# BAMresearch/PGDrome

Measured on AMD Instinct MI355X. Metric: PGD fixed-point iters/sec + SpMV HBM GB/s, 256^3 P1 space x 1D param, higher is better.
Workload: dtype f64

## Files before the change

### include/pgd_amd.h

```cpp
#ifndef PGD_AMD_H
#define PGD_AMD_H

#include <stdint.h>

#ifdef __cplusplus
extern "C" {
#endif

typedef int64_t pgd_handle;

enum {
    PGD_OK = 0,
    PGD_ERR_INVALID = -1,
    PGD_ERR_HIP = -2,
    PGD_ERR_NOMEM = -3,
    PGD_ERR_LIMIT = -4,
    PGD_ERR_SINGULAR = -5,
    PGD_ERR_NODEVICE = -6,
    PGD_ERR_TIMEOUT = -7,
    PGD_ERR_PEER = -8
};

enum {
    PGD_ATOM_MASS = 0,
// ... 89 lines not shown
int pgd_slots_upload(pgd_handle ctx, const double *in, int first, int count);
int pgd_flags_reset(pgd_handle ctx);
int pgd_flags_download(pgd_handle ctx, int32_t *done, int32_t *iters, int32_t *status);
int pgd_op_diag_inv(pgd_handle ctx, pgd_handle op, pgd_handle dinv);
int pgd_op_symmetrize(pgd_handle ctx, pgd_handle op, int *used);
int pgd_atom_product_form(pgd_handle ctx, pgd_handle A, int *form);

int pgd_op_classify(pgd_handle ctx, pgd_handle op, int *classes);
int pgd_spmv_dot_slot(pgd_handle ctx, pgd_handle A, pgd_handle x, pgd_handle y, pgd_handle w,
                      int64_t r0, int64_t r1, int slot);
int pgd_pcg_init_slot(pgd_handle ctx, pgd_handle b, pgd_handle q, pgd_handle dinv, pgd_handle r,
                      pgd_handle z, pgd_handle p, int64_t r0, int64_t r1, int slot);
int pgd_pcg_tol_slot(pgd_handle ctx, double rtol, double atol, int slot_rr, int slot_bb,
                     int slot_tol2);
int pgd_pcg_xr_slot(pgd_handle ctx, pgd_handle x, pgd_handle r, pgd_handle p, pgd_handle q,
                    pgd_handle dinv, pgd_handle z, int64_t r0, int64_t r1, int slot_rz,
                    int slot_pq, int slot_out);
int pgd_pcg_check_slot(pgd_handle ctx, int slot_rr, int slot_tol2);
int pgd_pcg_p_slot(pgd_handle ctx, pgd_handle p, pgd_handle z, int64_t r0, int64_t r1,
                   int slot_num, int slot_den);

int pgd_cg_init_slot(pgd_handle ctx, pgd_handle b, pgd_handle q, pgd_handle dinv, pgd_handle r,
                     pgd_handle u, pgd_handle p, pgd_handle s, int64_t r0, int64_t r1, int base);
int pgd_cg_update_slot(pgd_handle ctx, pgd_handle x, pgd_handle r, pgd_handle u, pgd_handle w,
                       pgd_handle p, pgd_handle s, pgd_handle dinv, int64_t r0, int64_t r1, int base);
int pgd_cg_scalars_slot(pgd_handle ctx, int base, int init, double rtol, double atol);

typedef int (*pgd_halo_fn)(void *user, pgd_handle vec, int64_t own0, int64_t own1, int64_t lo_ghost,
                           int64_t hi_ghost);
typedef int (*pgd_allreduce_fn)(void *user, int first_slot, int count);
int pgd_comm_bind_callbacks(pgd_handle ctx, pgd_halo_fn halo, pgd_allreduce_fn allreduce, void *user,
                            int rank, int world);
int pgd_comm_unique_id(pgd_handle ctx, uint8_t *out128);
int pgd_comm_bind_rccl(pgd_handle ctx, const uint8_t *id128, int rank, int world);
int pgd_comm_overlap(pgd_handle ctx, int mode, int *state);
int pgd_comm_unbind(pgd_handle ctx);
int pgd_comm_timeout(pgd_handle ctx, double seconds);
int pgd_comm_prof(pgd_handle ctx, int mode, double *out8);
int pgd_comm_info(pgd_handle ctx, int *kind , int *rank, int *world);
int pgd_comm_halo(pgd_handle ctx, pgd_handle vec, int64_t own0, int64_t own1, int64_t lo_ghost,
                  int64_t hi_ghost);
int pgd_comm_allreduce_slots(pgd_handle ctx, int first_slot, int count);

#define PGD_PUSH_BLOB_BYTES 256
int pgd_comm_push_export(pgd_handle ctx, int64_t n, int64_t own0, int64_t own1, int64_t lo_ghost, int64_t hi_ghost,
                         uint8_t *blob );
int pgd_comm_push_attach(pgd_handle ctx, const uint8_t *lower_blob, const uint8_t *upper_blob, int *state);
int pgd_comm_push(pgd_handle ctx, int mode, int *state);
int pgd_comm_allreduce_attach(pgd_handle ctx, const uint8_t *all_blobs, int *state);
int pgd_comm_allreduce_direct(pgd_handle ctx, int mode, int *state);
int pgd_pcg_solve_sharded(pgd_handle ctx, pgd_handle A, pgd_handle b, pgd_handle x, int64_t own0,
                          int64_t own1, int64_t lo_ghost, int64_t hi_ghost, double rtol, double atol,
                          int maxit, int *iters, double *rel_res);

int pgd_bicgstab_solve(pgd_handle ctx, pgd_handle A, pgd_handle b, pgd_handle x, double rtol, double atol,
                       int maxit, int *iters, double *rel_res);

int pgd_start_gram(pgd_handle ctx, pgd_handle A, const pgd_handle *vecs, int k, pgd_handle b, int64_t r0,
                   int64_t r1, double *out);
int pgd_start_residual(pgd_handle ctx, pgd_handle A, int k, const double *coefs, pgd_handle b, pgd_handle r);

int pgd_vec_multidot(pgd_handle ctx, pgd_handle x, const pgd_handle *ys, int k, int64_t lo, int64_t hi,
                     double *out);

int pgd_vec_multidot_pair(pgd_handle ctx, pgd_handle x0, pgd_handle x1, const pgd_handle *ys, int k, int64_t lo,
                          int64_t hi, double *out);

enum { PGD_BLOCK_F32 = 0, PGD_BLOCK_F64 = 1 };
int pgd_block_create(pgd_handle ctx, int64_t n, int k, int dtype, pgd_handle *block);
int pgd_block_free(pgd_handle ctx, pgd_handle block);
int pgd_block_info(pgd_handle ctx, pgd_handle block, int64_t *n, int *k, int *dtype, int64_t *bytes);
int pgd_block_storage(pgd_handle ctx, int *dtype);
int pgd_block_set_column(pgd_handle ctx, pgd_handle block, int j, pgd_handle vec);
int pgd_block_get_column(pgd_handle ctx, pgd_handle block, int j, pgd_handle vec);
int pgd_block_dots(pgd_handle ctx, pgd_handle block, pgd_handle vec_r, int64_t lo, int64_t hi, double *out);
int pgd_block_combine(pgd_handle ctx, pgd_handle block, const double *coefs, pgd_handle vec_base_or_0, pgd_handle vec_x);

enum { PGD_EVAL_STATS = 1, PGD_EVAL_ENVELOPE = 2, PGD_EVAL_EXCEED = 4, PGD_EVAL_FIELDS = 8 };
int pgd_eval_batch(pgd_handle ctx, const pgd_handle *modes, int k, const double *coefs, int64_t s, int want,
                   double threshold, double *sample_stats, pgd_handle env_min, pgd_handle env_max, pgd_handle exceed,
                   pgd_handle fields);

enum {
    PGD_TUNE_BLOCK_STORAGE = 54,
    PGD_TUNE_PCG_RECOMPUTE_Q = 53,
    PGD_TUNE_EVAL_SAMPLE_CHUNK = 52,
    PGD_TUNE_EVAL_GRID_MAX = 51,
    PGD_TUNE_EVAL_VARIANT = 50,
    PGD_TUNE_PUSH_IN_UPDATE = 49,
    PGD_TUNE_STENCIL_ROWS = 48,
    PGD_TUNE_DIA_MARCH3 = 47,
    PGD_TUNE_SHARD_ONE_MARCH = 46,
    PGD_TUNE_HALO_OVERLAP_MIN_ROWS = 45,
    PGD_TUNE_COMM_SELF_PERIODIC = 44,
    PGD_TUNE_PCG_DERIVE_SCALED = 43,
    PGD_TUNE_MG_MARCH_MIN = 42,
    PGD_TUNE_MG_CHUNK = 41,
    PGD_TUNE_PCG_PRECOND = 40,
    PGD_TUNE_CLS_CACHE = 39,
    PGD_TUNE_STENCIL_DEPTH = 38,
    PGD_TUNE_STENCIL_WG_PER_CU = 37,
    PGD_TUNE_SPMV_ZCHUNK_STENCIL = 36,
    PGD_TUNE_SPMV_STENCIL = 35,
    PGD_TUNE_FAULT_STALL_MS = 34,
    PGD_TUNE_FAULT_STAGE = 33,
    PGD_TUNE_SPMV_ZCHUNK_CODED2 = 32,
    PGD_TUNE_PCG_PIPELINE = 31,
    PGD_TUNE_PCG_EXACT_PHASE = 30,
    PGD_TUNE_PCG_FOLD_FINISH = 29,
    PGD_TUNE_LAZY_CSR = 28,
    PGD_TUNE_ATOM_FAST = 27,
    PGD_TUNE_SPMV_ROWS = 1,
    PGD_TUNE_SPMV_GRID_MIN_BYTES = 8,
    PGD_TUNE_PCG_FOLD_REDUCE = 12,
    PGD_TUNE_PCG_SCALED = 10,
    PGD_TUNE_SPMV_ZCHUNK_FORCE = 7,
    PGD_TUNE_PCG_SMALL_ROWS = 26,
    PGD_TUNE_PCG_SMALL_SINGLE_SYNC = 25,
    PGD_TUNE_SPMV_FETCH_DEPTH = 24,
    PGD_TUNE_PCG_STREAM_HINTS = 23,
    PGD_TUNE_PCG_LAG_X = 22,
    PGD_TUNE_SPMV_ZCHUNK_CODED = 21,
    PGD_TUNE_ASM_LATTICE = 20,
    PGD_TUNE_SPMV_ROW_CLASSES = 19,
    PGD_TUNE_PCG_SINGLE_SYNC = 18,
    PGD_TUNE_UNIT_DIAG = 17,
    PGD_TUNE_PCG_DEFER_X = 16,
    PGD_TUNE_FAULT_ITERATION = 15,
    PGD_TUNE_COMBINE_DIA = 14,
    PGD_TUNE_SPMV_VARIANT = 13,
    PGD_TUNE_SPMV_ZCHUNK = 6,
    PGD_TUNE_SPMV_SYM = 3,
    PGD_TUNE_SPMV_DICT = 2
};
int pgd_tune(pgd_handle ctx, int knob, int64_t value);

int pgd_prof_enable(pgd_handle ctx, int on);
int pgd_prof_read(pgd_handle ctx, int64_t *launches, double *seconds, double *alg_bytes);
int pgd_prof_read_own(pgd_handle ctx, double *own_bytes);
int pgd_prof_read_update(pgd_handle ctx, int64_t *launches, double *seconds, double *bytes);
int pgd_prof_read_dropped(pgd_handle ctx, int64_t *dropped);
int pgd_prof_event_overhead(pgd_handle ctx, double *seconds);
int pgd_kernel_counts(pgd_handle ctx, int64_t *out, int n);
int pgd_pcg_recompute_counts(pgd_handle ctx, int64_t *updates);
int pgd_classify_counts(pgd_handle ctx, int64_t *full, int64_t *cached);
int pgd_mg_counts(pgd_handle ctx, int64_t *solves, int64_t *fallbacks);
int pgd_vmg_counts(pgd_handle ctx, int64_t *solves, int64_t *fallbacks, int64_t *levels);
int pgd_vmg_times(pgd_handle ctx, double *setup_ms, int64_t *march_passes);
int pgd_cmg_counts(pgd_handle ctx, int64_t *solves, int64_t *fallbacks, int64_t *levels);
int pgd_cmg_times(pgd_handle ctx, double *setup_ms, int64_t *march_passes);
int pgd_mg_slab_setup(pgd_handle ctx, pgd_handle A, int nz_global, int z_first, int64_t own0, int64_t own1,
                      int64_t *n_coarse, int *applies);
int pgd_mg_slab_fix_start(pgd_handle ctx, pgd_handle A, pgd_handle b, pgd_handle x, int64_t own0, int64_t own1);
int pgd_mg_slab_down(pgd_handle ctx, pgd_handle r, pgd_handle t);
int pgd_mg_slab_restrict(pgd_handle ctx, pgd_handle t, pgd_handle b1);
int pgd_mg_coarse(pgd_handle ctx, pgd_handle b1, pgd_handle x1);
int pgd_mg_slab_up(pgd_handle ctx, pgd_handle r, pgd_handle x1, pgd_handle t, pgd_handle z, int slot, double *dot);
int pgd_calib_stream(pgd_handle ctx, pgd_handle vec, int bytes_per_lane, int store);
int pgd_timer_start(pgd_handle ctx);
int pgd_timer_stop(pgd_handle ctx, double *seconds);

#ifdef __cplusplus
}
#endif
#endif
```

### pgdrome_amd/_lib.py

```python
from __future__ import annotations

import ctypes as C
from pathlib import Path

import numpy as np

LIB_PATH = Path(__file__).resolve().parent / "lib" / "libpgd_amd.so"

H = C.c_int64
I64 = C.c_int64
I32 = C.c_int32
F64 = C.c_double
PD = C.POINTER(C.c_double)
PI32 = C.POINTER(C.c_int32)
PI64 = C.POINTER(C.c_int64)
PH = C.POINTER(C.c_int64)
VP = C.c_void_p

PU8 = C.POINTER(C.c_uint8)
HALO_FN = C.CFUNCTYPE(C.c_int, VP, H, I64, I64, I64, I64)
ALLREDUCE_FN = C.CFUNCTYPE(C.c_int, VP, C.c_int, C.c_int)

SIGNATURES = {
    "pgd_ctx_create": (C.c_int, [C.c_int, VP, PH]),
# ... 38 lines not shown
    "pgd_atom_assemble": (C.c_int, [H, H, C.c_int, C.c_int, C.c_int, H, PH]),
    "pgd_atom_assemble_cells": (C.c_int, [H, H, C.c_int, C.c_int, C.c_int, H, PU8, I64, PH]),
    "pgd_atom_assemble_cellwise": (C.c_int, [H, H, C.c_int, C.c_int, C.c_int, H, H, PU8, I64, PH]),
    "pgd_atom_assemble_facets": (C.c_int, [H, H, PI32, I64, C.c_int, PH]),
    "pgd_atom_upload": (C.c_int, [H, H, PD, PH]),
    "pgd_atom_download": (C.c_int, [H, H, PD]),
    "pgd_atom_free": (C.c_int, [H, H]),
    "pgd_op_combine": (C.c_int, [H, H, PH, PD, C.c_int, PI32, I64, PH]),
    "pgd_spmv": (C.c_int, [H, H, H, H, I64, I64]),
    "pgd_bilinear": (C.c_int, [H, H, H, H, I64, I64, PD]),
    "pgd_bilinear_many": (C.c_int, [H, H, H, PH, C.c_int, I64, I64, PD]),
    "pgd_start_gram": (C.c_int, [H, H, PH, C.c_int, H, I64, I64, PD]),
    "pgd_start_residual": (C.c_int, [H, H, C.c_int, PD, H, H]),
    "pgd_mg_slab_setup": (C.c_int, [H, H, C.c_int, C.c_int, I64, I64, C.POINTER(I64), C.POINTER(C.c_int)]),
    "pgd_mg_slab_fix_start": (C.c_int, [H, H, H, H, I64, I64]),
    "pgd_mg_slab_down": (C.c_int, [H, H, H]),
    "pgd_mg_slab_restrict": (C.c_int, [H, H, H]),
    "pgd_mg_coarse": (C.c_int, [H, H, H]),
    "pgd_mg_slab_up": (C.c_int, [H, H, H, H, H, C.c_int, PD]),
    "pgd_bicgstab_solve": (C.c_int, [H, H, H, H, C.c_double, C.c_double, C.c_int, C.POINTER(C.c_int), PD]),
    "pgd_atom_product_form": (C.c_int, [H, H, C.POINTER(C.c_int)]),
    "pgd_vec_multidot": (C.c_int, [H, H, PH, C.c_int, I64, I64, PD]),
    "pgd_vec_multidot_pair": (C.c_int, [H, H, H, PH, C.c_int, I64, I64, PD]),
    "pgd_pcg_solve": (C.c_int, [H, H, H, H, F64, F64, C.c_int, C.POINTER(C.c_int), PD]),
    "pgd_pcg_last_form": (C.c_int, [H, C.POINTER(C.c_int), C.POINTER(C.c_int)]),
    "pgd_band_solve": (C.c_int, [H, H, H, H]),
    "pgd_slots_ptr": (C.c_int, [H, C.POINTER(VP)]),
    "pgd_slots_download": (C.c_int, [H, PD, C.c_int, C.c_int]),
    "pgd_slots_upload": (C.c_int, [H, PD, C.c_int, C.c_int]),
    "pgd_flags_reset": (C.c_int, [H]),
    "pgd_flags_download": (C.c_int, [H, PI32, PI32, PI32]),
    "pgd_op_diag_inv": (C.c_int, [H, H, H]),
    "pgd_spmv_dot_slot": (C.c_int, [H, H, H, H, H, I64, I64, C.c_int]),
    "pgd_pcg_init_slot": (C.c_int, [H, H, H, H, H, H, H, I64, I64, C.c_int]),
    "pgd_pcg_tol_slot": (C.c_int, [H, F64, F64, C.c_int, C.c_int, C.c_int]),
    "pgd_pcg_xr_slot": (C.c_int, [H, H, H, H, H, H, H, I64, I64, C.c_int, C.c_int, C.c_int]),
    "pgd_pcg_check_slot": (C.c_int, [H, C.c_int, C.c_int]),
    "pgd_pcg_p_slot": (C.c_int, [H, H, H, I64, I64, C.c_int, C.c_int]),
    "pgd_cg_init_slot": (C.c_int, [H, H, H, H, H, H, H, H, I64, I64, C.c_int]),
    "pgd_cg_update_slot": (C.c_int, [H, H, H, H, H, H, H, H, I64, I64, C.c_int]),
    "pgd_cg_scalars_slot": (C.c_int, [H, C.c_int, C.c_int, F64, F64]),
    "pgd_comm_bind_callbacks": (C.c_int, [H, HALO_FN, ALLREDUCE_FN, VP, C.c_int, C.c_int]),
    "pgd_comm_unique_id": (C.c_int, [H, PU8]),
    "pgd_comm_bind_rccl": (C.c_int, [H, PU8, C.c_int, C.c_int]),
    "pgd_comm_overlap": (C.c_int, [H, C.c_int, C.POINTER(C.c_int)]),
    "pgd_comm_unbind": (C.c_int, [H]),
    "pgd_comm_timeout": (C.c_int, [H, F64]),
    "pgd_comm_prof": (C.c_int, [H, C.c_int, PD]),
    "pgd_comm_info": (C.c_int, [H, C.POINTER(C.c_int), C.POINTER(C.c_int), C.POINTER(C.c_int)]),
    "pgd_comm_halo": (C.c_int, [H, H, I64, I64, I64, I64]),
    "pgd_comm_allreduce_slots": (C.c_int, [H, C.c_int, C.c_int]),
    "pgd_comm_push_export": (C.c_int, [H, I64, I64, I64, I64, I64, PU8]),
    "pgd_comm_push_attach": (C.c_int, [H, PU8, PU8, C.POINTER(C.c_int)]),
    "pgd_comm_push": (C.c_int, [H, C.c_int, C.POINTER(C.c_int)]),
    "pgd_comm_allreduce_attach": (C.c_int, [H, PU8, C.POINTER(C.c_int)]),
    "pgd_comm_allreduce_direct": (C.c_int, [H, C.c_int, C.POINTER(C.c_int)]),
    "pgd_pcg_solve_sharded": (C.c_int, [H, H, H, H, I64, I64, I64, I64, F64, F64, C.c_int, C.POINTER(C.c_int), PD]),
    "pgd_op_symmetrize": (C.c_int, [H, H, C.POINTER(C.c_int)]),
    "pgd_op_classify": (C.c_int, [H, H, C.POINTER(C.c_int)]),
    "pgd_tune": (C.c_int, [H, C.c_int, I64]),
    "pgd_prof_enable": (C.c_int, [H, C.c_int]),
    "pgd_prof_read": (C.c_int, [H, PI64, PD, PD]),
    "pgd_prof_read_own": (C.c_int, [H, PD]),
    "pgd_prof_read_update": (C.c_int, [H, PI64, PD, PD]),
    "pgd_prof_read_dropped": (C.c_int, [H, PI64]),
    "pgd_prof_event_overhead": (C.c_int, [H, PD]),
    "pgd_kernel_counts": (C.c_int, [H, PI64, C.c_int]),
    "pgd_pcg_recompute_counts": (C.c_int, [H, PI64]),
    "pgd_classify_counts": (C.c_int, [H, PI64, PI64]),
    "pgd_mg_counts": (C.c_int, [H, PI64, PI64]),
    "pgd_vmg_counts": (C.c_int, [H, PI64, PI64, PI64]),
    "pgd_vmg_times": (C.c_int, [H, C.POINTER(C.c_double), PI64]),
    "pgd_cmg_counts": (C.c_int, [H, PI64, PI64, PI64]),
    "pgd_cmg_times": (C.c_int, [H, C.POINTER(C.c_double), PI64]),
    "pgd_calib_stream": (C.c_int, [H, H, C.c_int, C.c_int]),
    "pgd_timer_start": (C.c_int, [H]),
    "pgd_timer_stop": (C.c_int, [H, PD]),
}

NSLOTS = 64
EVAL_STATS, EVAL_ENVELOPE, EVAL_EXCEED, EVAL_FIELDS = 1, 2, 4, 8
TUNE_EVAL_VARIANT, TUNE_EVAL_GRID_MAX, TUNE_EVAL_SAMPLE_CHUNK = 50, 51, 52
TUNE_BLOCK_STORAGE = 54
BLOCK_F32, BLOCK_F64, BLOCK_MAXK = 0, 1, 64


ERR_TIMEOUT, ERR_PEER = -7, -8


class PgdError(RuntimeError):
    def __init__(self, code, msg):
        super().__init__(f"libpgd_amd error {code}: {msg}")
        self.code = code


_lib = None


def load(path: Path | None = None):
    global _lib
    if _lib is not None and path is None:
        return _lib
    p = Path(path) if path else LIB_PATH
    if not p.exists():
        raise RuntimeError(
            f"{p} not found: build the HIP library first (python -m pgdrome_amd.build). "
            "pgdrome_amd has no CPU fallback.")
    _preload_hip_runtime()
    lib = C.CDLL(str(p))
    for name, (res, args) in SIGNATURES.items():
        fn = getattr(lib, name)
        fn.restype = res
        fn.argtypes = args
    if path is None:
        _lib = lib
    return lib


def _preload_hip_runtime():
    import importlib.util
    try:
        spec = importlib.util.find_spec("torch")
    except (ImportError, ValueError):
        spec = None
    if spec is None or not spec.submodule_search_locations:
        return
    cand = Path(list(spec.submodule_search_locations)[0]) / "lib" / "libamdhip64.so"
    if cand.exists():
        try:
            C.CDLL(str(cand), mode=C.RTLD_GLOBAL)
        except OSError:
            pass


def dptr(a: np.ndarray):
    assert a.dtype == np.float64 and a.flags.c_contiguous
    return a.ctypes.data_as(PD)


def iptr(a: np.ndarray):
    assert a.dtype == np.int32 and a.flags.c_contiguous
    return a.ctypes.data_as(PI32)


class Context:

    def __init__(self, device: int = 0, stream: int | None = None):
        self.lib = load()
        if self.lib.pgd_device_count() <= 0:
            raise RuntimeError("pgdrome_amd: no HIP device visible (no CPU fallback exists)")
        h = H(0)
        rc = self.lib.pgd_ctx_create(device, VP(stream) if stream else None, C.byref(h))
        if rc != 0:
            raise PgdError(rc, self.lib.pgd_last_error(0).decode())
        self.h = h.value
        self.device = device
        self._block_k = {}

    def close(self):
        if getattr(self, "h", 0):
            self.lib.pgd_ctx_destroy(self.h)
            self.h = 0

    def __del__(self):
        try:
            self.close()
# ... 598 lines not shown
```

### pgdrome_amd/csrc/pgd_internal.h

```cpp
#pragma once

#include <hip/hip_runtime.h>

#include <chrono>
#include <cstdint>
#include <cstdio>
#include <map>
#include <memory>
#include <string>
#include <vector>

#include "../../include/pgd_amd.h"

namespace pgd {

constexpr int WAVE = 64;
constexpr int TPB = 256;
constexpr int MAX_VEC_BLOCKS = 2048;
constexpr int N_XCD = 8;
constexpr int DICT_MAXP = 256;
constexpr int DICT_DLEN = 32;
constexpr size_t PAD_BYTES = 256;

enum { S_PQ = 2, S_TOL2 = 5, S_DMIN = 7 , S_TMP = 8  };
enum { S1_RZ = 24, S1_RR = 25, S1_ALPHA = 26, S1_BETA = 27, S1_PQ = 28, S1_QQ = 29,
       S1_ALPHA_PREV = 40, S1_BETA_PREV = 41, S1_PEND = 42 };
constexpr double LAG_MIN_BETA = 0.01;

struct Ctx;
void dev_release(Ctx *c, void *p, size_t bytes);

struct Obj {
    enum Kind { FREE = 0, VEC, MESH, CSR, BLOCK } kind = FREE;
    Ctx *ctx = nullptr;
    uint64_t serial = 0;
    virtual ~Obj() {}
};

struct Vec : Obj {
    double *d = nullptr;
    int64_t n = 0;
    ~Vec() override { if (d) dev_release(ctx, d, (size_t)(n > 0 ? n : 1) * sizeof(double)); }
};

struct Block : Obj {
    void *d = nullptr;
    int64_t n = 0, stride = 0;
    int k = 0, dtype = 0;
    size_t bytes = 0;
    ~Block() override { if (d) dev_release(ctx, d, bytes); }
};

struct Mesh : Obj {
    int gdim = 0, nvpc = 0;
    int ncomp = 1;
    pgd_handle base = 0;
    int64_t nv = 0, nc = 0, nnz = 0;
    double *coords = nullptr;
    int4 *cells = nullptr;
    int *cellsN = nullptr;
    int *v2c_ptr = nullptr;
    int *v2c = nullptr;
    int *row_ptr = nullptr;
    int *cols = nullptr;
    int max_row = 0, kl = 0, ku = 0;
    int *sym_tab = nullptr;
    int sym_w = 0;
    int sym_nx = 0, sym_ny = 0;
    bool lattice = false;
    bool lattice_unit = false;
    bool lattice_regular = false;
    int pat_off[6][4] = {{0}};
    int pat_loc[6][8] = {{0}};
    double lat_h[3] = {0.0, 0.0, 0.0};
    struct ClsCache {
        uint64_t sig = 0; int scaled = 0, z_lo = 0, z_hi = 0, ncls = 0;
        uint8_t *codes = nullptr; int *same = nullptr; int *reps = nullptr; size_t bytes = 0;
        bool st_ok = false; int ident = -1, base = -1, zm0 = 0, zm1 = 0;
        uint8_t zero_pat[256];
        uint8_t in_range[256];
        uint64_t used = 0;
    };
    mutable std::vector<ClsCache> cls_cache;
    mutable uint64_t cls_clock = 0;
    std::vector<int32_t> bc_host;
    int *bc_dev = nullptr;
    size_t bc_dev_bytes = 0;
    uint16_t *pids = nullptr;
    int *dict_off = nullptr;
    int dict_count = 0;
    ~Mesh() override {
        for (void *p : {(void *)coords, (void *)cells, (void *)cellsN, (void *)v2c_ptr, (void *)v2c,
                        (void *)row_ptr, (void *)cols, (void *)pids, (void *)dict_off, (void *)sym_tab})
            if (p) (void)hipFree(p);
        for (ClsCache &e : cls_cache) if (e.same) (void)hipFree(e.same);
        if (bc_dev) (void)hipFree(bc_dev);
    }
};

struct Csr : Obj {
    pgd_handle mesh = 0;
    double *vals = nullptr;
    double *dinv = nullptr;
    bool dinv_valid = false;
    double *uvals = nullptr;
    bool uvals_valid = false;
    bool uvals_scaled = false;
    bool uvals_unit = false;
    int64_t uvals_stride = 0;
// ... 36 lines not shown
    void *nccl = nullptr;
    void *nccl_halo = nullptr;
    hipStream_t halo_stream = nullptr;
    hipEvent_t ev_ready = nullptr, ev_halo = nullptr;
    bool overlap = false;
    int64_t overlap_min_rows = (int64_t)1 << 40;
    bool overlap_used = false;
    bool self_periodic = false;
    pgd_handle work[7] = {0, 0, 0, 0, 0, 0, 0};
    int64_t work_n = 0;
    double timeout_s = 60.0;
    int *snap_flags = nullptr;
    double *snap_vote = nullptr;
    hipEvent_t snap_ev[2] = {nullptr, nullptr};
    bool prof = false;
    hipEvent_t mark[2][7] = {{nullptr, nullptr, nullptr, nullptr, nullptr, nullptr, nullptr}, {nullptr, nullptr, nullptr, nullptr, nullptr, nullptr, nullptr}};
    bool mark_set[2] = {false, false};
    double prof_sum[8] = {0, 0, 0, 0, 0, 0, 0, 0};
    bool push = false;
    bool push_used = false;
    int64_t push_n = 0, push_own0 = 0, push_own1 = 0, push_lo_g = 0, push_hi_g = 0;
    double *push_peer[2] = {nullptr, nullptr};
    int64_t push_peer_n[2] = {0, 0};
    unsigned long long *push_flags = nullptr;
    unsigned long long *push_peer_flags[2] = {nullptr, nullptr};
    void *push_mapped[4] = {nullptr, nullptr, nullptr, nullptr};
    unsigned long long push_seq = 0;
    bool ar = false, ar_used = false;
    unsigned long long *ar_peer[16] = {nullptr, nullptr, nullptr, nullptr, nullptr, nullptr, nullptr, nullptr,
                                       nullptr, nullptr, nullptr, nullptr, nullptr, nullptr, nullptr, nullptr};
    void *ar_mapped[16] = {nullptr, nullptr, nullptr, nullptr, nullptr, nullptr, nullptr, nullptr,
                           nullptr, nullptr, nullptr, nullptr, nullptr, nullptr, nullptr, nullptr};
    unsigned long long ar_seq = 0;
};
constexpr int PUSH_BLOCK_BYTES = 4096, PUSH_AR_FLAG0 = 8, PUSH_BOX_OFF = 512, PUSH_AR_MAXW = 16;

struct Ctx {
    int device = 0;
    hipStream_t stream = nullptr;
    bool own_stream = false;
    std::string err;
    std::vector<std::unique_ptr<Obj>> objs;
    std::vector<int64_t> free_list;

    std::multimap<size_t, void *> pool;
    size_t pool_bytes = 0;
    static constexpr size_t POOL_MAX = (size_t)24 << 30;

    double *slots = nullptr;
    int *flags = nullptr;
    double *partials = nullptr;
    int64_t partials_cap = 0;
    int64_t partials_off = 0;
    double *work[7] = {nullptr, nullptr, nullptr, nullptr, nullptr, nullptr, nullptr};
    int64_t work_cap[7] = {0, 0, 0, 0, 0, 0, 0};
    uint8_t *mask = nullptr;
    int64_t mask_cap = 0;
    int *ibuf = nullptr;
    int64_t ibuf_cap = 0;
    std::vector<int32_t> set_idx_host;
    std::vector<double> set_val_host;
    int *set_idx = nullptr;
    double *set_vals = nullptr;
    int64_t set_idx_cap = 0, set_vals_cap = 0;
    int32_t set_idx_max = 0;
    bool set_idx_on_dev = false, set_val_on_dev = false;

    Comm comm;

    int num_cu = 256;
    int spmv_dict = 1;
    int spmv_rows = 64;
    int64_t spmv_grid_min_plane_bytes = 0;
    int spmv_zchunk_force = 0;
    int fault_iteration = -1;
    int fault_stage = 0;
    int fault_stall_ms = 0;
    int64_t pcg_small_ss_rows = (int64_t)1 << 22;
    int pcg_small_ss = 1;
    int pcg_stream_hints = 1;
    int pcg_lag_x = 1;
    int pcg_recompute_q = 1;
    int64_t pcg_recompute_launches = 0;
    int asm_lattice = 1;
    int spmv_fetch_depth = 6;
    int spmv_zchunk_coded2 = 96;
    int spmv_zchunk_coded = 24;
    int pcg_exact_phase = 1;
    int pcg_fold_finish = 1;
    int atom_fast = 1;
    int lazy_csr = 1;
    uint64_t next_serial = 1;
    int pcg_precond = 0;
    struct Mg *mg = nullptr;
    struct Mg *mg_slab = nullptr;
    int64_t mg_solves = 0, mg_fallbacks = 0;
    struct Vmg *vmg = nullptr;
    int64_t vmg_solves = 0, vmg_fallbacks = 0, vmg_marches = 0;
    double vmg_setup_ms = 0.0;
    struct Cmg *cmg = nullptr;
    int64_t cmg_solves = 0, cmg_fallbacks = 0, cmg_marches = 0;
    double cmg_setup_ms = 0.0;
    int eval_variant = 1, eval_grid_max = 0, eval_chunk = 0;
    double *eval_pin = nullptr;
    size_t eval_pin_bytes = 0;
    hipEvent_t eval_ev[2] = {nullptr, nullptr};
    bool eval_ev_set[2] = {false, false};
    int mg_chunk = 2;
    int mg_march_min = 64;
    int cls_cache_on = 1;
    int64_t cls_fast = 0, cls_full = 0;
    int spmv_stencil = 1;
    int spmv_zchunk_stencil = 0;
    int stencil_depth = 0;
    int stencil_wg_per_cu = 2;
    int spmv_classes = 1;
    void *cls_scratch = nullptr;
    double *gram_w = nullptr;
    size_t gram_w_bytes = 0;
    pgd_handle gram_op = 0;
    int gram_k = 0;
    int64_t gram_n = 0;
    int spmv_variant = 0;
    int spmv_zchunk = 8;
    int pcg_fold_reduce = 1;
    int spmv_qq = 0;
    int pcg_single_sync = 1;
    int spmv_unit_diag = 1;
    int pcg_defer_x = 1;
    int pcg_scaled = 1;
    int stencil_rows = 0;
    int dia_march3 = 0;
    int push_in_update = 1;
    int shard_one_march = 1;
    int pcg_derive_scaled = 1;
    int spmv_combine_dia = 1;
    int spmv_sym = 1;
    int block_storage = 1;

    bool prof = false;
    bool prof_pcg_only = false;
    std::vector<hipEvent_t> ev;
    struct ProfRec { uint8_t kind; int iter; double bytes, own, seconds; };
    std::vector<ProfRec> ev_rec;
    std::vector<ProfRec> prof_pend;
    int prof_iter = -1;
    int64_t prof_dropped = 0;
    double prof_overhead = -1.0;
    size_t ev_used = 0;
    int64_t prof_upd_launches = 0, prof_upd_seen = 0;
    double prof_upd_seconds = 0.0, prof_upd_bytes = 0.0;
    int64_t prof_launches = 0, prof_seen = 0;
    double prof_seconds = 0.0, prof_bytes = 0.0;
    double prof_own_bytes = 0.0;
    int64_t kcount[8] = {0, 0, 0, 0, 0, 0, 0, 0};
    hipEvent_t timer_ev[2] = {nullptr, nullptr};
    int *flags_host = nullptr;
    hipEvent_t flag_ev[2] = {nullptr, nullptr};
    int pcg_pipeline = 1;
    int pcg_last_form = -1, pcg_last_precond = -1;
};

struct ProfIterGuard { Ctx *c; ~ProfIterGuard() { c->prof_iter = -1; } };
inline double host_now() { return std::chrono::duration<double>(std::chrono::steady_clock::now().time_since_epoch()).count(); }

enum { KC_CSR = 0, KC_CSR_DICT = 1, KC_SYM_ROWS = 2, KC_DIA_ROWS = 3, KC_DIA_MARCH = 4, KC_MULTI = 5, KC_DIAC_MARCH = 6, KC_STENCIL_MARCH = 7 };

Ctx *get_ctx(pgd_handle h);
int fail(Ctx *c, int code, const char *fmt, ...);
pgd_handle put_obj(Ctx *c, Obj *o);
Obj *get_obj(Ctx *c, pgd_handle h, Obj::Kind k);
int free_obj(Ctx *c, pgd_handle h, Obj::Kind k);
int dev_alloc(Ctx *c, void **p, size_t bytes);
int ensure_partials(Ctx *c, int64_t n);
int ensure_work(Ctx *c, int i, int64_t n);
int ensure_mask(Ctx *c, int64_t n);
int pcg_flag_snapshots(Ctx *c);
int ensure_ibuf(Ctx *c, int64_t n);
void prof_flush(Ctx *c);
void prof_commit(Ctx *c, int valid_products, int valid_updates);
void comm_release(Ctx *c);
struct Mesh;
struct Csr;
int build_sym_tables(Ctx *c, Mesh *m);
int ensure_sym(Ctx *c, const Mesh *m, Csr *a, bool *usable);
int cg_init_s(Ctx *c, const double *b, const double *q, const double *sc, double *r, double *p, double *s, int64_t lo,
              int64_t hi, int base);
int cg_update_s(Ctx *c, double *x, double *r, const double *w, double *p, double *s, const double *sc, int64_t lo, int64_t hi,
                int base);
int cg_update_s2(Ctx *c, double *x, double *r, const double *w, double *p, double *s, const double *sc, int64_t lo, int64_t hi,
                 int base, int parity, int *nblocks);
int reduce_two_slots(Ctx *c, int na, int nb, int base);
int pcg1_seed(Ctx *c, int npairs, int slot_rz, int slot_rr);
int pcg1_tol(Ctx *c, int base, double rtol, double atol, int slot_p8);
int pcg1_aux(Ctx *c, const double *s, const double *r, int64_t lo, int64_t hi, int slot);
int pcg1_sums(Ctx *c, int nprod, int nvec, int base);
int pcg1_finish_slots(Ctx *c, int base);
struct PushArgs {
    double *dst_lo = nullptr, *dst_hi = nullptr;
    int64_t lo_end = 0, hi_begin = 0;
    unsigned long long *post_lo = nullptr, *post_hi = nullptr;
    const unsigned long long *wait_a = nullptr, *wait_b = nullptr;
    unsigned long long seq = 0, *ticket = nullptr;
    unsigned int nblocks = 0;
    long long ticks = 0;
};
unsigned int pcg1_update_push_blocks(int g, int64_t lo, int64_t hi, int64_t lo_end, int64_t hi_begin);
int pcg1_update(Ctx *c, double *x, double *r, double *p, const double *q, const double *sc, int64_t lo, int64_t hi, int base,
                int *nblocks, int lag, int fold_par, const PushArgs *push = nullptr);
int pcg1_flush_x(Ctx *c, double *x, const double *p, const double *r, int64_t lo, int64_t hi, int base, int fold_par);
int vec_sqrt(Ctx *c, double *v, int64_t n);
int vec_div_mul(Ctx *c, double *x, const double *sc, int64_t n, int mul);
int ensure_vals(Ctx *c, const Mesh *m, Csr *a);
bool atom_fast_form(Ctx *c, const Mesh *m, Csr *a, int64_t r0, int64_t r1);
int dia_classify(Ctx *c, const Mesh *m, Csr *a, int zrange_lo = -1, int zrange_hi = -1);
bool stencil_row_range(const Ctx *c, const Mesh *m, const Csr *a, int64_t r0, int64_t r1);
bool stencil_whole_grid(const Ctx *c, const Mesh *m, const Csr *a);
int stencil_update_blocks(const Ctx *c, const Mesh *m);
int launch_stencil_update(Ctx *c, const Mesh *m, const Csr *a, const double *p_in, double *p_out, double *x, double *r, const double *s,
                          double *pairs, int lag);
int launch_stencil_pass(Ctx *c, const uint8_t *cls, int ident, const double cst[8], int nx, int ny, int nz, int zm0, int zm1,
                        const double *x, const double *b, double *y, double w, int epi, bool dot, int *nparts, int z0 = 0, int z1 = -1);
bool mg_prepare(Ctx *c, const Mesh *m, const Csr *a);
int mg_fix_start(Ctx *c, const Csr *a, const double *b, double *x, int64_t n);
int mg_vcycle(Ctx *c, const double *r, bool dot, int *nparts, double *z_out = nullptr);
double *mg_result(Ctx *c);
void mg_release(Ctx *c);
struct Vmg;
bool vmg_prepare(Ctx *c, Vmg *&M, const Mesh *m, const Csr *a);
int vmg_fix_start(Ctx *c, Vmg *M, const double *sc, const double *b, double *x, int64_t n);
int vmg_vcycle(Ctx *c, Vmg *M, const double *r, bool dot, int *nparts, double *z_out, int64_t *marches);
double *vmg_result(Vmg *M);
void vmg_note_setup(Ctx *c);
void vmg_release(Ctx *c);
bool cmg_prepare(Ctx *c, const Mesh *m, const Mesh *base, const Csr *a);
int cmg_fix_start(Ctx *c, const double *b, double *x, int64_t n);
int cmg_apply(Ctx *c, const double *r, double *z, int64_t n, int *nparts);
void cmg_note_setup(Ctx *c);
void eval_release(Ctx *c);
int sym_scale(Ctx *c, const Mesh *m, Csr *a, const double *s);
int launch_spmv_dia_rows2(Ctx *c, const Mesh *m, const Csr *a, const double *x, double *y, const double *w, int64_t r0a,
                          int64_t r1a, int64_t r0b, int64_t r1b, bool dot, const int *flags, int *nparts_out, bool *done);
int combine_dia(Ctx *c, const Mesh *m, Csr *o, Csr *const *atoms, const double *coefs, int n, const uint8_t *mask);
int launch_spmv_op(Ctx *c, const Mesh *m, const Csr *a, const double *x, double *y, const double *w, int64_t r0,
                   int64_t r1, bool dot, bool store, const int *flags, int *nparts_out);

inline Vec *get_vec(Ctx *c, pgd_handle h) { return static_cast<Vec *>(get_obj(c, h, Obj::VEC)); }
inline Mesh *get_mesh(Ctx *c, pgd_handle h) { return static_cast<Mesh *>(get_obj(c, h, Obj::MESH)); }
inline Csr *get_csr(Ctx *c, pgd_handle h) { return static_cast<Csr *>(get_obj(c, h, Obj::CSR)); }
inline Block *get_block(Ctx *c, pgd_handle h) { return static_cast<Block *>(get_obj(c, h, Obj::BLOCK)); }

#define PGD_CTX(c, h)                         \
    pgd::Ctx *c = pgd::get_ctx(h);            \
    if (!c) return PGD_ERR_INVALID;           \
    (void)hipSetDevice(c->device)

#define PGD_HIP(c, call)                                                                    \
    do {                                                                                    \
        hipError_t e_ = (call);                                                             \
        if (e_ != hipSuccess)                                                               \
            return pgd::fail(c, PGD_ERR_HIP, "%s failed: %s (%s:%d)", #call,                \
                             hipGetErrorString(e_), __FILE__, __LINE__);                    \
    } while (0)

#define PGD_TRY(call)                \
    do {                             \
        int rc_ = (call);            \
        if (rc_ != PGD_OK) return rc_; \
    } while (0)

#define PGD_LAUNCH_CHECK(c) PGD_HIP(c, hipGetLastError())

inline int grid_for(int64_t n, int per_block = TPB, int cap = MAX_VEC_BLOCKS) {
    int64_t g = (n + per_block - 1) / per_block;
    if (g < 1) g = 1;
    if (g > cap) g = cap;
    return (int)g;
}

int scan_exclusive_i32(Ctx *c, const int *in, int *out, int64_t n);
int reduce_partials(Ctx *c, const double *partials, int nparts, int nvals, int slot0, int check_mode,
                    int slot_rr, int slot_tol2);
int reduce_partials_to(Ctx *c, const double *partials, int nparts, int nvals, double *dest, int blocks = 1);
int k_reduce_stage1_pub(Ctx *c, const double *partials, int nparts, int nvals, double *out);
int vec_dot_range(Ctx *c, const double *x, const double *y, int64_t lo, int64_t hi, int slot);
int launch_spmv(Ctx *c, const Mesh *m, const double *vals, const double *x, double *y,
                const double *w, int64_t r0, int64_t r1, bool dot, bool store, const int *flags,
                int *nparts_out);
int launch_spmv_multi(Ctx *c, const Mesh *m, const double *vals, const double *x,
                      const double *const *ys, int ny, int64_t r0, int64_t r1, double *out_host);
int csr_diag_inv(Ctx *c, const Mesh *m, Csr *a);

}

namespace pgd {

__device__ __forceinline__ int xcd_remap(int bid, int nblk) {
    const int q = nblk >> 3, rem = nblk & 7, k = bid & 7;
    return k * q + (k < rem ? k : rem) + (bid >> 3);
}

__device__ __forceinline__ double wave_sum(double v) {
#pragma unroll
    for (int off = 32; off > 0; off >>= 1) v += __shfl_down(v, off, 64);
    return v;
}

template <int NW>
__device__ __forceinline__ double block_sum_n(double v, double *s_red ) {
    v = wave_sum(v);
    if (NW == 1) return v;
    const int lane = threadIdx.x & 63, wv = threadIdx.x >> 6;
    __syncthreads();
    if (lane == 0) s_red[wv] = v;
    __syncthreads();
    double t = 0.0;
    if (threadIdx.x == 0) {
#pragma unroll
        for (int k = 0; k < NW; ++k) t += s_red[k];
    }
    return t;
}

__device__ __forceinline__ double block_sum(double v, double *s_red ) {
    v = wave_sum(v);
    const int lane = threadIdx.x & 63, wv = threadIdx.x >> 6;
    __syncthreads();
    if (lane == 0) s_red[wv] = v;
    __syncthreads();
    return (threadIdx.x == 0) ? ((s_red[0] + s_red[1]) + (s_red[2] + s_red[3])) : 0.0;
}

}
```

### pgdrome_amd/csrc/pgd_pcg.hip

```cpp
#include "pgd_internal.h"

#include <cmath>

#include <cstring>

#include <algorithm>

namespace pgd {

constexpr int MAXT = 8;
constexpr int CHECK_EVERY = 16;
constexpr int PROF_EAGER_EVERY = 8;

struct CombineArgs {
    const double *in[MAXT];
    double coef[MAXT];
    int n;
};

__global__ __launch_bounds__(TPB) void k_combine(CombineArgs A, double *__restrict__ out, const int *__restrict__ cols,
                                                 const uint8_t *__restrict__ colmask, int64_t nnz) {
    for (int64_t k = (int64_t)blockIdx.x * TPB + threadIdx.x; k < nnz; k += (int64_t)gridDim.x * TPB) {
        double s = 0.0;
#pragma unroll
// ... 321 lines not shown
                                                    double *__restrict__ x, int n, int kl, int ku,
                                                    double *__restrict__ gwork, int use_lds, int *__restrict__ flags) {
    __shared__ double s_w[BAND_LDS_DOUBLES];
    const int ld = 2 * kl + ku + 1;
    double *W = use_lds ? s_w : gwork;
    double *rhs = W + (int64_t)n * ld;
    for (int64_t k = threadIdx.x; k < (int64_t)n * ld; k += TPB) W[k] = 0.0;
    __syncthreads();
    for (int i = threadIdx.x; i < n; i += TPB) {
        rhs[i] = b[i];
        for (int k = row_ptr[i]; k < row_ptr[i + 1]; ++k) {
            const int j = cols[k];
            W[(i - j + kl + ku) + (int64_t)j * ld] = vals[k];
        }
    }
    __syncthreads();
    if (threadIdx.x == 0) {
        const int kv = kl + ku;
        int singular = 0;
        for (int j = 0; j < n; ++j) {
            const int imax = min(j + kl, n - 1), cmax = min(j + kv, n - 1);
            int piv = j;
            double best = fabs(W[kv + (int64_t)j * ld]);
            for (int i = j + 1; i <= imax; ++i) {
                const double t = fabs(W[(i - j + kv) + (int64_t)j * ld]);
                if (t > best) { best = t; piv = i; }
            }
            if (best == 0.0) { singular = 1; break; }
            if (piv != j) {
                for (int cc = j; cc <= cmax; ++cc) {
                    const int64_t a1 = (j - cc + kv) + (int64_t)cc * ld, a2 = (piv - cc + kv) + (int64_t)cc * ld;
                    const double t = W[a1]; W[a1] = W[a2]; W[a2] = t;
                }
                const double t = rhs[j]; rhs[j] = rhs[piv]; rhs[piv] = t;
            }
            const double dinv = 1.0 / W[kv + (int64_t)j * ld];
            for (int i = j + 1; i <= imax; ++i) {
                const double l = W[(i - j + kv) + (int64_t)j * ld] * dinv;
                if (l != 0.0) {
                    for (int cc = j + 1; cc <= cmax; ++cc)
                        W[(i - cc + kv) + (int64_t)cc * ld] -= l * W[(j - cc + kv) + (int64_t)cc * ld];
                    rhs[i] -= l * rhs[j];
                }
            }
        }
        if (!singular) {
            for (int j = n - 1; j >= 0; --j) {
                const int cmax = min(j + kv, n - 1);
                double s = rhs[j];
                for (int cc = j + 1; cc <= cmax; ++cc) s -= W[(j - cc + kv) + (int64_t)cc * ld] * rhs[cc];
                rhs[j] = s / W[kv + (int64_t)j * ld];
            }
        } else {
            flags[2] = PGD_ERR_SINGULAR;
        }
    }
    __syncthreads();
    for (int i = threadIdx.x; i < n; i += TPB) x[i] = rhs[i];
}


__global__ __launch_bounds__(TPB) void k_scale_in(const double *__restrict__ dinv, double *__restrict__ s,
                                                  double *__restrict__ x, int64_t n, unsigned long long *__restrict__ dmax_bits) {
    double mx = 0.0;
    for (int64_t i = (int64_t)blockIdx.x * TPB + threadIdx.x; i < n; i += (int64_t)gridDim.x * TPB) {
        const double di = dinv[i], si = sqrt(di);
        s[i] = si;
        x[i] = x[i] / si;
        mx = fmax(mx, di);
    }
    for (int o = 32; o > 0; o >>= 1) mx = fmax(mx, __shfl_xor(mx, o));
    if ((threadIdx.x & 63) == 0) {
        const unsigned long long mine = (unsigned long long)__double_as_longlong(mx);
        if (mine > __hip_atomic_load(dmax_bits, __ATOMIC_RELAXED, __HIP_MEMORY_SCOPE_AGENT)) atomicMax(dmax_bits, mine);
    }
}

struct StencilTuple { double c[8]; };
__global__ void k_stencil_derive(StencilTuple A, int unit, double *__restrict__ out) {
    if (threadIdx.x != 0 || blockIdx.x != 0) return;
    const double dinv = 1.0 / A.c[0], si = sqrt(dinv);
    out[0] = unit ? 1.0 : A.c[0] * si * si;
    for (int s = 1; s < 8; ++s) { double v = A.c[s]; v *= si * si; out[s] = v; }
}

__global__ void k_dmin_slot(const unsigned long long *__restrict__ dmax_bits, double *__restrict__ slots, int *__restrict__ flags) {
    const double dmax_inv = __longlong_as_double((long long)dmax_bits[0]);
    slots[S_DMIN] = dmax_inv > 0.0 ? 1.0 / dmax_inv : 0.0;
    if (!(dmax_inv > 0.0) || !(dmax_inv < 1e300)) { flags[0] = 1; flags[2] = PGD_ERR_SINGULAR; }
}

__global__ __launch_bounds__(TPB) void k_pcg_init_s(const double *__restrict__ b, const double *__restrict__ q,
                                                    const double *__restrict__ s, double *__restrict__ r,
                                                    double *__restrict__ p, int64_t n, double *__restrict__ partials) {
    __shared__ double s_red[4];
    double rz = 0.0, rr = 0.0, bb = 0.0;
    for (int64_t i = (int64_t)blockIdx.x * TPB + threadIdx.x; i < n; i += (int64_t)gridDim.x * TPB) {
        const double bi = b[i], si = s[i], ri = si * bi - q[i], ti = ri / si;
        r[i] = ri; p[i] = ri;
        rz = fma(ri, ri, rz); rr = fma(ti, ti, rr); bb = fma(bi, bi, bb);
    }
    rz = block_sum(rz, s_red);
    rr = block_sum(rr, s_red);
    bb = block_sum(bb, s_red);
    if (threadIdx.x == 0) {
        partials[3 * blockIdx.x + 0] = rz;
        partials[3 * blockIdx.x + 1] = rr;
        partials[3 * blockIdx.x + 2] = bb;
    }
}

__global__ __launch_bounds__(TPB) void k_pcg_xr_s(double *__restrict__ x, double *__restrict__ r, const double *__restrict__ p,
                                                  const double *__restrict__ q, const double *__restrict__ s, int64_t n,
                                                  const double *__restrict__ slots, int slot_rz, int slot_pq,
                                                  double *__restrict__ partials, const int *__restrict__ flags) {
    if (flags[0]) return;
    __shared__ double s_red[4];
    typedef double d2 __attribute__((ext_vector_type(2)));
    const double alpha = slots[slot_rz] / slots[slot_pq];
    const bool exact = flags[3] != 0;
    double rz = 0.0, rr = 0.0;
    const int64_t npair = n >> 1;
    for (int64_t k = (int64_t)blockIdx.x * TPB + threadIdx.x; k < npair; k += (int64_t)gridDim.x * TPB) {
        const int64_t i = 2 * k;
        const d2 pi = *reinterpret_cast<const d2 *>(p + i), qi = *reinterpret_cast<const d2 *>(q + i);
        d2 xi = *reinterpret_cast<d2 *>(x + i), ri = *reinterpret_cast<d2 *>(r + i);
        xi.x = fma(alpha, pi.x, xi.x); xi.y = fma(alpha, pi.y, xi.y);
        ri.x = fma(-alpha, qi.x, ri.x); ri.y = fma(-alpha, qi.y, ri.y);
        *reinterpret_cast<d2 *>(x + i) = xi;
        *reinterpret_cast<d2 *>(r + i) = ri;
        rz = fma(ri.x, ri.x, rz); rz = fma(ri.y, ri.y, rz);
        if (exact) {
            const d2 si = *reinterpret_cast<const d2 *>(s + i);
            const double tx = ri.x / si.x, ty = ri.y / si.y;
            rr = fma(tx, tx, rr); rr = fma(ty, ty, rr);
        }
    }
    if ((n & 1) && blockIdx.x == 0 && threadIdx.x == 0) {
        const int64_t i = n - 1;
        x[i] = fma(alpha, p[i], x[i]);
        const double ri = fma(-alpha, q[i], r[i]);
        r[i] = ri;
        rz = fma(ri, ri, rz);
        if (exact) { const double t = ri / s[i]; rr = fma(t, t, rr); }
    }
    rz = block_sum(rz, s_red);
    rr = block_sum(rr, s_red);
    if (threadIdx.x == 0) { partials[2 * blockIdx.x] = rz; partials[2 * blockIdx.x + 1] = exact ? rr : rz; }
}

__global__ __launch_bounds__(TPB) void k_pcg_r_s(double *__restrict__ r, const double *__restrict__ q, const double *__restrict__ s,
                                                 int64_t n, const double *__restrict__ slots, int slot_rz, int slot_pq,
                                                 double *__restrict__ partials, const int *__restrict__ flags) {
    if (flags[0]) return;
    __shared__ double s_red[4];
    typedef double d2 __attribute__((ext_vector_type(2)));
    const double alpha = slots[slot_rz] / slots[slot_pq];
    const bool exact = flags[3] != 0;
    double rz = 0.0, rr = 0.0;
    const int64_t npair = n >> 1;
    for (int64_t k = (int64_t)blockIdx.x * TPB + threadIdx.x; k < npair; k += (int64_t)gridDim.x * TPB) {
        const int64_t i = 2 * k;
        const d2 qi = *reinterpret_cast<const d2 *>(q + i);
        d2 ri = *reinterpret_cast<d2 *>(r + i);
        ri.x = fma(-alpha, qi.x, ri.x); ri.y = fma(-alpha, qi.y, ri.y);
        *reinterpret_cast<d2 *>(r + i) = ri;
        rz = fma(ri.x, ri.x, rz); rz = fma(ri.y, ri.y, rz);
        if (exact) {
            const d2 si = *reinterpret_cast<const d2 *>(s + i);
            const double tx = ri.x / si.x, ty = ri.y / si.y;
            rr = fma(tx, tx, rr); rr = fma(ty, ty, rr);
        }
    }
    if ((n & 1) && blockIdx.x == 0 && threadIdx.x == 0) {
        const int64_t i = n - 1;
        const double ri = fma(-alpha, q[i], r[i]);
        r[i] = ri;
        rz = fma(ri, ri, rz);
        if (exact) { const double t = ri / s[i]; rr = fma(t, t, rr); }
    }
    rz = block_sum(rz, s_red);
    rr = block_sum(rr, s_red);
    if (threadIdx.x == 0) { partials[2 * blockIdx.x] = rz; partials[2 * blockIdx.x + 1] = exact ? rr : rz; }
}

__global__ __launch_bounds__(TPB) void k_pcg_px_s(double *__restrict__ x, double *__restrict__ p, const double *__restrict__ r,
                                                  int64_t n, const double *__restrict__ slots, int slot_new, int slot_old,
                                                  int slot_pq, const int *__restrict__ flags) {
    if (flags[0]) return;
    typedef double d2 __attribute__((ext_vector_type(2)));
    const double alpha = slots[slot_old] / slots[slot_pq], beta = slots[slot_new] / slots[slot_old];
    const int64_t npair = n >> 1;
    for (int64_t k = (int64_t)blockIdx.x * TPB + threadIdx.x; k < npair; k += (int64_t)gridDim.x * TPB) {
        const int64_t i = 2 * k;
        const d2 ri = *reinterpret_cast<const d2 *>(r + i);
        d2 pi = *reinterpret_cast<d2 *>(p + i), xi = *reinterpret_cast<d2 *>(x + i);
        xi.x = fma(alpha, pi.x, xi.x); xi.y = fma(alpha, pi.y, xi.y);
        pi.x = fma(beta, pi.x, ri.x); pi.y = fma(beta, pi.y, ri.y);
        *reinterpret_cast<d2 *>(x + i) = xi;
        *reinterpret_cast<d2 *>(p + i) = pi;
    }
    if ((n & 1) && blockIdx.x == 0 && threadIdx.x == 0) {
        const int64_t i = n - 1;
        x[i] = fma(alpha, p[i], x[i]);
        p[i] = fma(beta, p[i], r[i]);
    }
}

enum { S1F_ALPHA = 44 , S1F_BETA = 46 , S1F_EXACT = 48  };

__device__ __forceinline__ void pcg1_finish(double *slots, int *flags, double pq, double qq, double rz, double rr, int slot_alpha,
                                            int slot_beta, bool keep_prev = false) {
    const double tol2 = slots[S_TOL2];
    if (!(rz == rz) || !(pq == pq)) { flags[0] = 1; flags[2] = PGD_ERR_SINGULAR; return; }
    if (flags[3]) { if (rr <= tol2) { flags[0] = 1; return; } }
    else if (rz * slots[S_DMIN] <= 1e4 * tol2) flags[3] = 1;
    if (!(rz > 0.0)) { flags[0] = 1; return; }
    const double alpha = rz / pq;
    double rnew = alpha * alpha * qq - rz;
    if (!(rnew > 0.0)) rnew = 0.0;
    if (keep_prev) { slots[S1_ALPHA_PREV] = slots[slot_alpha]; slots[S1_BETA_PREV] = slots[slot_beta]; }
    slots[slot_alpha] = alpha;
    slots[slot_beta] = rnew / rz;
    flags[1] += 1;
}

__global__ __launch_bounds__(1024) void k_pcg1_scalars(const double *__restrict__ prod, int nprod, const double *__restrict__ vecp,
                                                       int nvec, double *__restrict__ slots, int *__restrict__ flags) {
    __shared__ double s_w[16];
    if (flags[0]) return;
    const int lane = threadIdx.x & 63, wv = threadIdx.x >> 6;
    {
        const int v = wv >> 2, t = threadIdx.x & 255;
        const double *src = v < 2 ? prod : vecp;
        const int n = v < 2 ? nprod : nvec, off = v & 1;
        double a8[8] = {0, 0, 0, 0, 0, 0, 0, 0};
        int i = t;
        for (; i + 7 * 256 < n; i += 8 * 256) {
#pragma unroll
            for (int u = 0; u < 8; ++u) a8[u] += src[2 * (int64_t)(i + u * 256) + off];
        }
        for (int u = 0; i < n; i += 256, ++u) a8[u & 7] += src[2 * (int64_t)i + off];
        const double acc = wave_sum(((a8[0] + a8[1]) + (a8[2] + a8[3])) + ((a8[4] + a8[5]) + (a8[6] + a8[7])));
        if (lane == 0) s_w[wv] = acc;
    }
    __syncthreads();
    double out[4];
#pragma unroll
    for (int v = 0; v < 4; ++v) out[v] = (s_w[4 * v] + s_w[4 * v + 1]) + (s_w[4 * v + 2] + s_w[4 * v + 3]);
    if (threadIdx.x != 0) return;
    slots[S1_PQ] = out[0]; slots[S1_QQ] = out[1]; slots[S1_RZ] = out[2]; slots[S1_RR] = out[3];
    pcg1_finish(slots, flags, out[0], out[1], out[2], out[3], S1_ALPHA, S1_BETA, true);
}

__global__ __launch_bounds__(1024) void k_pcg1_sums(const double *__restrict__ prod, int nprod, const double *__restrict__ vecp,
                                                    int nvec, double *__restrict__ slots, int base, const int *__restrict__ flags) {
    __shared__ double s_w[16];
    if (flags[0]) return;
    const int lane = threadIdx.x & 63, wv = threadIdx.x >> 6;
    const int v = wv >> 2, t = threadIdx.x & 255;
    const double *src = v < 2 ? prod : vecp;
    const int n = v < 2 ? nprod : nvec, off = v & 1;
    double a8[8] = {0, 0, 0, 0, 0, 0, 0, 0};
    int i = t;
    for (; i + 7 * 256 < n; i += 8 * 256) {
#pragma unroll
        for (int u = 0; u < 8; ++u) a8[u] += src[2 * (int64_t)(i + u * 256) + off];
    }
    for (int u = 0; i < n; i += 256, ++u) a8[u & 7] += src[2 * (int64_t)i + off];
    const double acc = wave_sum(((a8[0] + a8[1]) + (a8[2] + a8[3])) + ((a8[4] + a8[5]) + (a8[6] + a8[7])));
    if (lane == 0) s_w[wv] = acc;
    __syncthreads();
    if (threadIdx.x < 4) slots[base + threadIdx.x] = (s_w[4 * threadIdx.x] + s_w[4 * threadIdx.x + 1]) + (s_w[4 * threadIdx.x + 2] + s_w[4 * threadIdx.x + 3]);
    if (threadIdx.x == 4) slots[base + 4] = 0.0;
}

__global__ void k_pcg1_finish(double *__restrict__ slots, int *__restrict__ flags, int base) {
    if (threadIdx.x != 0 || blockIdx.x != 0 || flags[0]) return;
    slots[6] = slots[base + 3];
    pcg1_finish(slots, flags, slots[base], slots[base + 1], slots[base + 2], slots[base + 3], base + 5, base + 6, true);
}

__global__ void k_pcg1_tol(double *__restrict__ slots, int *__restrict__ flags, int base, double rtol, double atol, int slot_p8) {
    if (threadIdx.x != 0 || blockIdx.x != 0) return;
    const double t1 = rtol * rtol * slots[base + 8], t2 = atol * atol, rr = slots[base + 1];
    slots[S_TOL2] = t1 > t2 ? t1 : t2;
    slots[6] = rr;
    int exact = 1;
    if (slot_p8 >= 0) {
        const double p8 = slots[slot_p8];
        if (p8 > 0.0 && p8 < 1e300) { slots[S_DMIN] = 1.0 / sqrt(sqrt(sqrt(p8))); exact = 0; }
        slots[slot_p8] = 0.0;
// ... 59 lines not shown
        alpha = rz0 / pq;
        double rnew = alpha * alpha * qq - rz0;
        if (!(rnew > 0.0)) rnew = 0.0;
        beta = rnew / rz0;
        if (lead) { slots[S1F_ALPHA + par] = alpha; slots[S1F_BETA + par] = beta; flags[1] += 1; }
    } else {
        alpha = slots[slot_alpha];
        beta = slots[slot_beta];
    }
    const bool exact = FOLD ? fold_exact : flags[3] != 0;
    const bool skip_x = lag == 1 && beta >= LAG_MIN_BETA;
    const bool two = lag == 2 && slots[S1_PEND] != 0.0;
    const double alpha_p = two ? slots[FOLD ? S1F_ALPHA + (par ^ 1) : S1_ALPHA_PREV] : 0.0;
    const double ibeta_p = two ? 1.0 / slots[FOLD ? S1F_BETA + (par ^ 1) : S1_BETA_PREV] : 0.0;
    double rz = 0.0, rr = 0.0;
    int pushed = 0;
    if ((lo & 1) == 0) {
        const int64_t npair = (hi - lo) >> 1;
        for (int64_t k = (int64_t)blockIdx.x * TPB + threadIdx.x; k < npair; k += (int64_t)gridDim.x * TPB) {
            const int64_t i = lo + 2 * k;
            const d2 qi = NT ? __builtin_nontemporal_load(reinterpret_cast<const d2 *>(q + i)) : *reinterpret_cast<const d2 *>(q + i);
            d2 pi = *reinterpret_cast<d2 *>(p + i);
            d2 ri = NT ? __builtin_nontemporal_load(reinterpret_cast<d2 *>(r + i)) : *reinterpret_cast<d2 *>(r + i);
            if (!skip_x) {
                d2 xi = NT ? __builtin_nontemporal_load(reinterpret_cast<d2 *>(x + i)) : *reinterpret_cast<d2 *>(x + i);
                if (two) { xi.x = fma(alpha_p, (pi.x - ri.x) * ibeta_p, xi.x); xi.y = fma(alpha_p, (pi.y - ri.y) * ibeta_p, xi.y); }
                xi.x = fma(alpha, pi.x, xi.x); xi.y = fma(alpha, pi.y, xi.y);
                if (NT) __builtin_nontemporal_store(xi, reinterpret_cast<d2 *>(x + i)); else *reinterpret_cast<d2 *>(x + i) = xi;
            }
            ri.x = fma(-alpha, qi.x, ri.x); ri.y = fma(-alpha, qi.y, ri.y);
            pi.x = fma(beta, pi.x, ri.x); pi.y = fma(beta, pi.y, ri.y);
            if (NT) __builtin_nontemporal_store(ri, reinterpret_cast<d2 *>(r + i)); else *reinterpret_cast<d2 *>(r + i) = ri;
            *reinterpret_cast<d2 *>(p + i) = pi;
            if (PUSH) {
                if (i < P.lo_end) { push_store(P.dst_lo + (i - lo), pi.x); push_store(P.dst_lo + (i - lo) + 1, pi.y); pushed = 1; }
                if (i >= P.hi_begin) { push_store(P.dst_hi + (i - P.hi_begin), pi.x); push_store(P.dst_hi + (i - P.hi_begin) + 1, pi.y); pushed = 1; }
            }
            rz = fma(ri.x, ri.x, rz); rz = fma(ri.y, ri.y, rz);
            if (exact) {
                const d2 si = *reinterpret_cast<const d2 *>(s + i);
                const double tx = ri.x / si.x, ty = ri.y / si.y;
                rr = fma(tx, tx, rr); rr = fma(ty, ty, rr);
            }
        }
    }
    const int64_t tail0 = (lo & 1) == 0 ? lo + 2 * ((hi - lo) >> 1) : lo;
    for (int64_t i = tail0 + (int64_t)blockIdx.x * TPB + threadIdx.x; i < hi; i += (int64_t)gridDim.x * TPB) {
        const double pi = p[i], r0 = r[i];
        if (!skip_x) {
            double xi = x[i];
            if (two) xi = fma(alpha_p, (pi - r0) * ibeta_p, xi);
            x[i] = fma(alpha, pi, xi);
        }
        const double ri = fma(-alpha, q[i], r0);
        r[i] = ri;
        p[i] = fma(beta, pi, ri);
        rz = fma(ri, ri, rz);
        if (exact) { const double t = ri / s[i]; rr = fma(t, t, rr); }
    }
    rz = block_sum(rz, s_red);
    rr = block_sum(rr, s_red);
    if (threadIdx.x == 0) { partials[2 * blockIdx.x] = rz; partials[2 * blockIdx.x + 1] = exact ? rr : rz; }
    if (lag == 1 && blockIdx.x == 0 && threadIdx.x == 0) slots[S1_PEND] = skip_x ? 1.0 : 0.0;
    if (PUSH) {
        __builtin_amdgcn_s_waitcnt(0);
        if (!__syncthreads_or(pushed)) return;
        if (threadIdx.x != 0) return;
        const unsigned long long t = __hip_atomic_fetch_add(P.ticket, 1ull, __ATOMIC_RELAXED, __HIP_MEMORY_SCOPE_AGENT);
        if (t + 1 != P.nblocks) return;
        __hip_atomic_store(P.ticket, 0ull, __ATOMIC_RELAXED, __HIP_MEMORY_SCOPE_AGENT);
        push_post(P);
        const long long t0 = wall_clock64();
        for (int which = 0; which < 2; ++which) {
            const unsigned long long *f = which ? P.wait_b : P.wait_a;
            if (!f) continue;
            while (__hip_atomic_load(f, __ATOMIC_ACQUIRE, __HIP_MEMORY_SCOPE_SYSTEM) < P.seq) {
                if (wall_clock64() - t0 > P.ticks) { flags[2] = PGD_ERR_TIMEOUT; flags[0] = 1; return; }
                __builtin_amdgcn_s_sleep(4);
            }
        }
    }
}

struct Pcg1Scalars { double alpha, beta; int exact, done, status; double pq, qq, rz, rr; };

__device__ __forceinline__ Pcg1Scalars pcg1_wg_scalars(const double *__restrict__ prod, int nprod, const double *__restrict__ vecp, int nvec,
                                                       const double *__restrict__ slots, int exact_cur, double *s_w ) {
    typedef double d2 __attribute__((ext_vector_type(2)));
    const int t = threadIdx.x, lane = t & 63, wv = t >> 6;
    double a[4] = {0.0, 0.0, 0.0, 0.0};
    for (int i = t; i < nprod; i += 256) { const d2 v = *reinterpret_cast<const d2 *>(prod + 2 * (int64_t)i); a[0] += v.x; a[1] += v.y; }
    for (int i = t; i < nvec; i += 256) { const d2 v = *reinterpret_cast<const d2 *>(vecp + 2 * (int64_t)i); a[2] += v.x; a[3] += v.y; }
#pragma unroll
    for (int v = 0; v < 4; ++v) a[v] = wave_sum(a[v]);
    __syncthreads();
    if (lane == 0) {
#pragma unroll
        for (int v = 0; v < 4; ++v) s_w[4 * v + wv] = a[v];
    }
    __syncthreads();
    double out[4];
#pragma unroll
    for (int v = 0; v < 4; ++v) out[v] = (s_w[4 * v] + s_w[4 * v + 1]) + (s_w[4 * v + 2] + s_w[4 * v + 3]);
    __syncthreads();
    Pcg1Scalars S;
    S.pq = out[0]; S.qq = out[1]; S.rz = out[2]; S.rr = out[3];
    S.alpha = S.beta = 0.0; S.exact = exact_cur; S.done = 0; S.status = 0;
    const double tol2 = slots[S_TOL2];
    if (!(S.rz == S.rz) || !(S.pq == S.pq)) { S.done = 1; S.status = PGD_ERR_SINGULAR; return S; }
    if (exact_cur) { if (S.rr <= tol2) { S.done = 1; return S; } }
    else if (S.rz * slots[S_DMIN] <= 1e4 * tol2) S.exact = 1;
    if (!(S.rz > 0.0)) { S.done = 1; return S; }
    S.alpha = S.rz / S.pq;
    double rnew = S.alpha * S.alpha * S.qq - S.rz;
    if (!(rnew > 0.0)) rnew = 0.0;
    S.beta = rnew / S.rz;
    return S;
}

__global__ __launch_bounds__(TPB) void k_pcg1_step(double *__restrict__ x, double *__restrict__ r, double *__restrict__ p,
                                                   const double *__restrict__ q, const double *__restrict__ s, int64_t n,
                                                   const double *__restrict__ prod, int nprod, const double *__restrict__ vec_in, int nvec,
                                                   double *__restrict__ vec_out, double *__restrict__ slots, int *__restrict__ flags,
                                                   int par, int lag) {
    __shared__ double s_red[16];
    __shared__ int s_done;
    if (threadIdx.x == 0) s_done = flags[0];
    __syncthreads();
    if (s_done) return;
    typedef double d2 __attribute__((ext_vector_type(2)));
    const Pcg1Scalars S = pcg1_wg_scalars(prod, nprod, vec_in, nvec, slots, slots[S1F_EXACT + (par ^ 1)] != 0.0, s_red);
    if (blockIdx.x == 0 && threadIdx.x == 0) {
        slots[S1_PQ] = S.pq; slots[S1_QQ] = S.qq; slots[S1_RZ] = S.rz; slots[S1_RR] = S.rr;
        slots[S1F_EXACT + par] = S.exact ? 1.0 : 0.0;
        flags[3] = S.exact;
        if (S.done) { if (S.status) flags[2] = S.status; flags[0] = 1; }
        else { slots[S1F_ALPHA + par] = S.alpha; slots[S1F_BETA + par] = S.beta; flags[1] += 1; }
    }
    if (S.done) return;
    const double alpha = S.alpha, beta = S.beta;
    const bool exact = S.exact != 0;
    const bool skip_x = lag == 1 && beta >= LAG_MIN_BETA;
    const bool two = lag == 2 && slots[S1_PEND] != 0.0;
    const double alpha_p = two ? slots[S1F_ALPHA + (par ^ 1)] : 0.0, ibeta_p = two ? 1.0 / slots[S1F_BETA + (par ^ 1)] : 0.0;
    double rz = 0.0, rr = 0.0;
    const int64_t npair = n >> 1;
    for (int64_t k = (int64_t)blockIdx.x * TPB + threadIdx.x; k < npair; k += (int64_t)gridDim.x * TPB) {
        const int64_t i = 2 * k;
        const d2 qi = *reinterpret_cast<const d2 *>(q + i);
        d2 pi = *reinterpret_cast<d2 *>(p + i), ri = *reinterpret_cast<d2 *>(r + i);
        if (!skip_x) {
            d2 xi = *reinterpret_cast<d2 *>(x + i);
            if (two) { xi.x = fma(alpha_p, (pi.x - ri.x) * ibeta_p, xi.x); xi.y = fma(alpha_p, (pi.y - ri.y) * ibeta_p, xi.y); }
            xi.x = fma(alpha, pi.x, xi.x); xi.y = fma(alpha, pi.y, xi.y);
            *reinterpret_cast<d2 *>(x + i) = xi;
        }
        ri.x = fma(-alpha, qi.x, ri.x); ri.y = fma(-alpha, qi.y, ri.y);
        pi.x = fma(beta, pi.x, ri.x); pi.y = fma(beta, pi.y, ri.y);
        *reinterpret_cast<d2 *>(r + i) = ri;
        *reinterpret_cast<d2 *>(p + i) = pi;
        rz = fma(ri.x, ri.x, rz); rz = fma(ri.y, ri.y, rz);
        if (exact) {
            const d2 si = *reinterpret_cast<const d2 *>(s + i);
            const double tx = ri.x / si.x, ty = ri.y / si.y;
            rr = fma(tx, tx, rr); rr = fma(ty, ty, rr);
        }
    }
    for (int64_t i = 2 * npair + (int64_t)blockIdx.x * TPB + threadIdx.x; i < n; i += (int64_t)gridDim.x * TPB) {
        const double pi = p[i], r0 = r[i];
        if (!skip_x) {
            double xi = x[i];
            if (two) xi = fma(alpha_p, (pi - r0) * ibeta_p, xi);
            x[i] = fma(alpha, pi, xi);
        }
        const double ri = fma(-alpha, q[i], r0);
        r[i] = ri;
        p[i] = fma(beta, pi, ri);
        rz = fma(ri, ri, rz);
        if (exact) { const double t = ri / s[i]; rr = fma(t, t, rr); }
    }
    rz = block_sum(rz, s_red);
    rr = block_sum(rr, s_red);
    if (threadIdx.x == 0) { vec_out[2 * blockIdx.x] = rz; vec_out[2 * blockIdx.x + 1] = exact ? rr : rz; }
    if (lag == 1 && blockIdx.x == 0 && threadIdx.x == 0) slots[S1_PEND] = skip_x ? 1.0 : 0.0;
}

__global__ void k_pcg1_seed(double *__restrict__ partials, int npairs, const double *__restrict__ slots, int slot_rz, int slot_rr) {
    for (int i = blockIdx.x * blockDim.x + threadIdx.x; i < npairs; i += gridDim.x * blockDim.x) {
        partials[2 * i] = i == 0 ? slots[slot_rz] : 0.0;
        partials[2 * i + 1] = i == 0 ? slots[slot_rr] : 0.0;
    }
}

__global__ __launch_bounds__(TPB) void k_scale_out(double *__restrict__ x, const double *__restrict__ r, const double *__restrict__ s,
                                                   int64_t n, double *__restrict__ partials, const double *__restrict__ p,
                                                   const double *__restrict__ slots, int slot_rz, int slot_pq, int lagged,
                                                   int slot_alpha, int slot_beta) {
    __shared__ double s_red[4];
    double rr = 0.0;
// ... 314 lines not shown
    *nblocks = 0;
    if (hi == lo) return push ? fail(c, PGD_ERR_INVALID, "pcg1_update: a push from an empty slab") : PGD_OK;
    const int g = grid_for((hi - lo + 1) / 2);
    PushArgs P;
    if (push) {
        if (fold_par < 0 || (lo & 1) || ((hi - lo) & 1) || ((push->lo_end - lo) & 1) || ((hi - push->hi_begin) & 1))
            return fail(c, PGD_ERR_INVALID, "pcg1_update: this launch cannot carry the direct halo");
        P = *push;
        if (!P.nblocks) P.nblocks = pcg1_update_push_blocks(g, lo, hi, P.lo_end, P.hi_begin);
    }
    PGD_TRY(ensure_work(c, 6, 2 * (int64_t)MAX_VEC_BLOCKS));
    bool timed_u;
    PGD_TRY(update_timing_begin(c, &timed_u));
    launch_pcg1_update(c, g, x, r, p, q, sc, lo, hi, base + 5, base + 6, c->work[6], lag, base, fold_par, push ? &P : nullptr);
    PGD_TRY(update_timing_end(c, timed_u, ((lag == 1 ? 40.0 : 56.0) + (c->pcg_exact_phase ? 0.0 : 8.0)) * (double)(hi - lo)));
    PGD_LAUNCH_CHECK(c);
    *nblocks = g;
    return PGD_OK;
}

__global__ __launch_bounds__(TPB) void k_pcg1_flush_x(double *__restrict__ x, const double *__restrict__ p, const double *__restrict__ r,
                                                      int64_t lo, int64_t hi, const double *__restrict__ slots, int slot_alpha,
                                                      int slot_beta) {
    if (slots[S1_PEND] == 0.0) return;
    const double alpha = slots[slot_alpha], ibeta = 1.0 / slots[slot_beta];
    for (int64_t i = lo + (int64_t)blockIdx.x * TPB + threadIdx.x; i < hi; i += (int64_t)gridDim.x * TPB)
        x[i] = fma(alpha, (p[i] - r[i]) * ibeta, x[i]);
}

int pcg1_flush_x(Ctx *c, double *x, const double *p, const double *r, int64_t lo, int64_t hi, int base, int fold_par) {
    if (hi == lo) return PGD_OK;
    const int sa = fold_par >= 0 ? S1F_ALPHA + fold_par : base + 5, sb = fold_par >= 0 ? S1F_BETA + fold_par : base + 6;
    k_pcg1_flush_x<<<grid_for(hi - lo), TPB, 0, c->stream>>>(x, p, r, lo, hi, c->slots, sa, sb);
    PGD_LAUNCH_CHECK(c);
    return PGD_OK;
}

static int pcg_xr(Ctx *c, double *x, double *r, const double *p, const double *q, const double *dinv, double *z,
                  int64_t lo, int64_t hi, int slot_rz, int slot_pq, int slot_out, int check_mode, int slot_tol2) {
    const int g = grid_for(hi - lo);
    const bool with_z = z != nullptr;
    PGD_TRY(ensure_partials(c, 4 * (int64_t)MAX_VEC_BLOCKS));
    if ((lo & 1) == 0) {
        const int g2 = grid_for((hi - lo + 1) / 2);
        if (with_z) k_pcg_xr<true><<<g2, TPB, 0, c->stream>>>(x, r, p, q, dinv, z, lo, hi, c->slots, slot_rz, slot_pq, c->partials, c->flags);
        else k_pcg_xr<true, false><<<g2, TPB, 0, c->stream>>>(x, r, p, q, nullptr, nullptr, lo, hi, c->slots, slot_rz, slot_pq, c->partials, c->flags);
        PGD_LAUNCH_CHECK(c);
        return reduce_partials(c, c->partials, g2, 2, slot_out, check_mode, slot_out + 1, slot_tol2);
    }
    if (with_z) k_pcg_xr<false><<<g, TPB, 0, c->stream>>>(x, r, p, q, dinv, z, lo, hi, c->slots, slot_rz, slot_pq, c->partials, c->flags);
    else k_pcg_xr<false, false><<<g, TPB, 0, c->stream>>>(x, r, p, q, nullptr, nullptr, lo, hi, c->slots, slot_rz, slot_pq, c->partials, c->flags);
    PGD_LAUNCH_CHECK(c);
    return reduce_partials(c, c->partials, g, 2, slot_out, check_mode, slot_out + 1, slot_tol2);
}

typedef pgd_pcg_form PcgForm;
typedef pgd_pcg_precond PcgPrecond;

static bool pcg_single_sync(PcgForm f) {
    return f == PGD_PCG_FORM_TWO_LAUNCH || f == PGD_PCG_FORM_SINGLE_SYNC || f == PGD_PCG_FORM_SINGLE_SYNC_RECOMPUTE;
}

static PcgForm pcg_choose(const Ctx *c, PcgPrecond precond, bool scaled, int64_t n, bool grid, bool whole) {
    const bool small = n <= ((int64_t)1 << 20);
    if (precond != PGD_PCG_PRECOND_JACOBI) return PGD_PCG_FORM_PRECOND;
    if (!scaled) return PGD_PCG_FORM_TEXTBOOK;
    if (c->pcg_single_sync && c->pcg_small_ss && (small || (grid && n <= c->pcg_small_ss_rows))) return PGD_PCG_FORM_TWO_LAUNCH;
    if (c->pcg_fold_reduce && small) return PGD_PCG_FORM_FOLDED;
    if (c->pcg_single_sync && grid) return (c->pcg_recompute_q && whole) ? PGD_PCG_FORM_SINGLE_SYNC_RECOMPUTE : PGD_PCG_FORM_SINGLE_SYNC;
    return c->pcg_defer_x ? PGD_PCG_FORM_DEFERRED_X : PGD_PCG_FORM_PLAIN;
}

struct PcgRun {
    static constexpr int S_INIT = 18, S_PAIR = 16;
    Ctx *c; const Mesh *m; Csr *o; const double *b; double *x; int64_t n;
    double *r, *z, *p, *q, *sc;
    double *part2 = nullptr, *part2b = nullptr;
    int gvec = 0, g2v = 0;
    PcgForm form = PGD_PCG_FORM_TEXTBOOK;
    PcgPrecond precond = PGD_PCG_PRECOND_JACOBI;
    bool scaled = false, lag_x = false;
    bool x_scaled = false;
    bool virt = false;
    double st_saved[8] = {0, 0, 0, 0, 0, 0, 0, 0};
    ~PcgRun() {
        if (virt) {
            for (int s2 = 0; s2 < 8; ++s2) o->st_c[s2] = st_saved[s2];
            o->st_virtual = false;
        }
        if (!x_scaled) return;
        (void)vec_div_mul(c, x, sc, n, 1);
        if (!virt) invalidate_slots();
    }
    void invalidate_slots() { o->uvals_valid = false; o->uvals_scaled = false; }
    int out(int k) const { return S_PAIR + 2 * (k & 1); }
    int old(int k) const { return S_PAIR + 2 * ((k + 1) & 1); }
    int g2() const { return grid_for((n + 1) / 2); }
};

static int pcg_precond_prepare(PcgRun &R) {
    Ctx *c = R.c;
    const Mesh *m = R.m;
    const int want = c->pcg_precond;
    if (want == 1 && R.scaled && mg_prepare(c, m, R.o)) { R.precond = PGD_PCG_PRECOND_MG; c->mg_solves += 1; return mg_fix_start(c, R.o, R.b, R.x, R.n); }
    if (want == 2 && R.scaled && m->sym_nx > 0 && vmg_prepare(c, c->vmg, m, R.o)) { R.precond = PGD_PCG_PRECOND_VMG; c->vmg_solves += 1; return vmg_fix_start(c, c->vmg, R.sc, R.b, R.x, R.n); }
    if (want == 3 && !R.scaled && m->ncomp >= 2) {
        PGD_TRY(ensure_vals(c, m, R.o));
        if (cmg_prepare(c, m, get_mesh(c, m->base), R.o)) { R.precond = PGD_PCG_PRECOND_CMG; c->cmg_solves += 1; return cmg_fix_start(c, R.b, R.x, R.n); }
    }
    if (want == 1) c->mg_fallbacks += 1;
    if (want == 2) c->vmg_fallbacks += 1;
    if (want == 3) c->cmg_fallbacks += 1;
    return PGD_OK;
}

static int pcg_precond_apply(PcgRun &R, const double *r, double *z_out, int *np) {
    switch (R.precond) {
    case PGD_PCG_PRECOND_MG: return mg_vcycle(R.c, r, true, np, z_out);
    case PGD_PCG_PRECOND_VMG: return vmg_vcycle(R.c, R.c->vmg, r, true, np, z_out, &R.c->vmg_marches);
    case PGD_PCG_PRECOND_CMG: return cmg_apply(R.c, r, z_out ? z_out : R.z, R.n, np);
    case PGD_PCG_PRECOND_JACOBI: break;
    }
    return fail(R.c, PGD_ERR_INVALID, "pcg_solve: no cycle to apply");
}
static double *pcg_precond_result(PcgRun &R) {
    return R.precond == PGD_PCG_PRECOND_MG ? mg_result(R.c) : R.precond == PGD_PCG_PRECOND_VMG ? vmg_result(R.c->vmg) : R.z;
}

static int pcg_derive_stencil(PcgRun &R) {
    Ctx *c = R.c;
    Csr *o = R.o;
    if (!(c->pcg_derive_scaled && R.m->sym_nx > 0 && c->pcg_precond != 2)) return PGD_OK;
    if (o->cls_count <= 0) PGD_TRY(dia_classify(c, R.m, o));
    if (!(stencil_whole_grid(c, R.m, o) && o->st_ident >= 0 && o->st_c[0] > 0.0)) return PGD_OK;
    PGD_TRY(ensure_work(c, 5, 4096));
    StencilTuple in;
    for (int s2 = 0; s2 < 8; ++s2) in.c[s2] = o->st_c[s2];
    k_stencil_derive<<<1, 1, 0, c->stream>>>(in, c->spmv_unit_diag, c->work[5] + 16);
    PGD_LAUNCH_CHECK(c);
    double out8[8];
    PGD_HIP(c, hipMemcpyAsync(out8, c->work[5] + 16, sizeof out8, hipMemcpyDeviceToHost, c->stream));
    PGD_HIP(c, hipStreamSynchronize(c->stream));
    for (double v : out8) if (!std::isfinite(v)) return PGD_OK;
    for (int s2 = 0; s2 < 8; ++s2) { R.st_saved[s2] = o->st_c[s2]; o->st_c[s2] = out8[s2]; }
    o->st_virtual = R.virt = true;
    return PGD_OK;
}

static int pcg_setup_scaled(PcgRun &R) {
    Ctx *c = R.c;
    const int64_t n = R.n;
    PGD_TRY(ensure_work(c, 5, 4096));
    unsigned long long *bits = reinterpret_cast<unsigned long long *>(c->work[5]);
    PGD_HIP(c, hipMemsetAsync(bits, 0, sizeof(unsigned long long), c->stream));
    k_scale_in<<<grid_for(n), TPB, 0, c->stream>>>(R.o->dinv, R.sc, R.x, n, bits);
    k_dmin_slot<<<1, 1, 0, c->stream>>>(bits, c->slots, c->flags);
    PGD_LAUNCH_CHECK(c);
    R.x_scaled = true;
    PGD_TRY(pcg_derive_stencil(R));
    if (!R.virt) {
        PGD_TRY(sym_scale(c, R.m, R.o, R.sc));
        PGD_TRY(dia_classify(c, R.m, R.o));
    }
    PGD_TRY(pcg_precond_prepare(R));
    PGD_TRY(launch_spmv_op(c, R.m, R.o, R.x, R.q, nullptr, 0, n, false, true, nullptr, nullptr));
    const int g = grid_for(n);
    PGD_TRY(ensure_partials(c, 4 * (int64_t)MAX_VEC_BLOCKS));
    k_pcg_init_s<<<g, TPB, 0, c->stream>>>(R.b, R.q, R.sc, R.r, R.p, n, c->partials);
    PGD_LAUNCH_CHECK(c);
    return reduce_partials(c, c->partials, g, 3, R.S_INIT, -1, 0, 0);
}

static int pcg_setup_unscaled(PcgRun &R) {
    PGD_TRY(pcg_precond_prepare(R));
    PGD_TRY(launch_spmv_op(R.c, R.m, R.o, R.x, R.q, nullptr, 0, R.n, false, true, nullptr, nullptr));
    return pcg_init(R.c, R.b, R.q, R.o->dinv, R.r, R.z, R.p, 0, R.n, R.S_INIT);
}

static int pcg_choose_and_seed(PcgRun &R) {
    Ctx *c = R.c;
    const int64_t n = R.n;
    if (R.precond != PGD_PCG_PRECOND_JACOBI) {
        int np = 0;
        PGD_TRY(pcg_precond_apply(R, R.r, R.p, &np));
        PGD_TRY(reduce_partials(c, c->partials, np, 1, R.S_INIT, -1, 0, 0));
    }
    PGD_TRY(ensure_work(c, 6, 4 * (int64_t)MAX_VEC_BLOCKS));
    c->pcg_last_precond = R.precond;
    c->pcg_last_form = R.form = pcg_choose(c, R.precond, R.scaled, n, R.m->sym_nx > 0, stencil_whole_grid(c, R.m, R.o));
    R.lag_x = c->pcg_lag_x && pcg_single_sync(R.form);
    R.g2v = grid_for((n + 1) / 2, TPB, (n > ((int64_t)1 << 20) && n <= c->pcg_small_ss_rows && c->pcg_small_ss) ? 512 : MAX_VEC_BLOCKS);
    R.gvec = R.form == PGD_PCG_FORM_SINGLE_SYNC_RECOMPUTE ? stencil_update_blocks(c, R.m) : R.g2v;
    if (2 * (int64_t)R.gvec > 4 * (int64_t)MAX_VEC_BLOCKS) PGD_TRY(ensure_work(c, 6, 2 * (int64_t)R.gvec));
    R.part2 = c->work[6];
    R.part2b = R.part2 + 2 * (int64_t)MAX_VEC_BLOCKS;
    if (!pcg_single_sync(R.form)) return PGD_OK;
    const bool two = R.form == PGD_PCG_FORM_TWO_LAUNCH;
    k_pcg1_seed<<<8, TPB, 0, c->stream>>>(two ? R.part2b : R.part2, R.gvec, c->slots, R.S_INIT, R.S_INIT + 1);
    if (two) PGD_HIP(c, hipMemsetAsync(c->slots + S1F_ALPHA, 0, 6 * sizeof(double), c->stream));
    PGD_LAUNCH_CHECK(c);
    return PGD_OK;
}

static int pcg_product(PcgRun &R, int *nparts, bool reduce = true) {
    PGD_TRY(launch_spmv_op(R.c, R.m, R.o, R.p, R.q, R.p, 0, R.n, true, true, R.c->flags, nparts));
    return reduce ? reduce_partials(R.c, R.c->partials, *nparts, 1, S_PQ, 0, 0, 0) : PGD_OK;
}
static int pcg_update_scaled(PcgRun &R, int k) {
    k_pcg_xr_s<<<R.g2(), TPB, 0, R.c->stream>>>(R.x, R.r, R.p, R.q, R.sc, R.n, R.c->slots, R.old(k), S_PQ, R.c->partials, R.c->flags);
    PGD_LAUNCH_CHECK(R.c);
    return reduce_partials(R.c, R.c->partials, R.g2(), 2, R.out(k), 2, R.out(k) + 1, S_TOL2);
}
static int pcg_update_unscaled(PcgRun &R, int k, double *z) {
    return pcg_xr(R.c, R.x, R.r, R.p, R.q, z ? R.o->dinv : nullptr, z, 0, R.n, R.old(k), S_PQ, R.out(k), 1, S_TOL2);
}
static void pcg_direction(PcgRun &R, int k, const double *z) {
    k_pcg_p<true><<<R.g2(), TPB, 0, R.c->stream>>>(R.p, z, 0, R.n, R.c->slots, R.out(k), R.old(k), R.c->flags);
}

static int pcg_iter_textbook(PcgRun &R, int k) {
    int nparts = 0;
    PGD_TRY(pcg_product(R, &nparts));
    PGD_TRY(pcg_update_unscaled(R, k, R.z));
    pcg_direction(R, k, R.z);
    return PGD_OK;
}

static int pcg_iter_plain(PcgRun &R, int k, int nparts = -1) {
    if (nparts < 0) PGD_TRY(pcg_product(R, &nparts));
    else PGD_TRY(reduce_partials(R.c, R.c->partials, nparts, 1, S_PQ, 0, 0, 0));
    PGD_TRY(pcg_update_scaled(R, k));
    pcg_direction(R, k, R.r);
    return PGD_OK;
}

static int pcg_iter_precond(PcgRun &R, int k) {
    int nparts = 0, np = 0;
    PGD_TRY(pcg_product(R, &nparts));
    PGD_TRY(R.precond == PGD_PCG_PRECOND_CMG ? pcg_update_unscaled(R, k, nullptr) : pcg_update_scaled(R, k));
    PGD_TRY(pcg_precond_apply(R, R.r, nullptr, &np));
    PGD_TRY(reduce_partials(R.c, R.c->partials, np, 1, R.out(k), -1, 0, 0));
    pcg_direction(R, k, pcg_precond_result(R));
    PGD_LAUNCH_CHECK(R.c);
    return PGD_OK;
}

static int pcg_iter_deferred_x(PcgRun &R, int k) {
    Ctx *c = R.c;
    int nparts = 0;
    PGD_TRY(pcg_product(R, &nparts));
    k_pcg_r_s<<<R.g2(), TPB, 0, c->stream>>>(R.r, R.q, R.sc, R.n, c->slots, R.old(k), S_PQ, c->partials, c->flags);
    PGD_LAUNCH_CHECK(c);
    PGD_TRY(reduce_partials(c, c->partials, R.g2(), 2, R.out(k), 2, R.out(k) + 1, S_TOL2));
    k_pcg_px_s<<<R.g2(), TPB, 0, c->stream>>>(R.x, R.p, R.r, R.n, c->slots, R.out(k), R.old(k), S_PQ, c->flags);
    return PGD_OK;
}

static int pcg_iter_folded(PcgRun &R, int k) {
    Ctx *c = R.c;
    int nparts = 0;
    PGD_TRY(pcg_product(R, &nparts, false));
    if (nparts <= 0 || nparts > 8192) return pcg_iter_plain(R, k, nparts);
    k_pcg_xr_s2<<<R.g2(), TPB, 0, c->stream>>>(R.x, R.r, R.p, R.q, R.sc, R.n, c->slots, R.old(k), c->partials, nparts, R.part2, c->flags);
    k_pcg_p_s2<<<R.g2(), TPB, 0, c->stream>>>(R.p, R.r, R.n, R.part2, R.g2(), c->slots, R.out(k), R.old(k), S_TOL2, c->flags);
    PGD_LAUNCH_CHECK(c);
    return PGD_OK;
}

struct Pcg1Iter { const double *prod; int nparts, lag; bool timed; };
static int pcg1_begin(PcgRun &R, int k, const double *p_cur, bool store, bool scalars, Pcg1Iter *I) {
    Ctx *c = R.c;
    I->lag = R.lag_x ? 1 + (k & 1) : 0;
    c->spmv_qq = 1;
    const int rc = launch_spmv_op(c, R.m, R.o, p_cur, R.q, p_cur, 0, R.n, true, store, c->flags, &I->nparts);
    c->spmv_qq = 0;
    PGD_TRY(rc);
    PGD_TRY(stage_product_partials(c, &I->prod, &I->nparts));
    if (scalars) k_pcg1_scalars<<<1, 1024, 0, c->stream>>>(I->prod, I->nparts, R.part2, R.gvec, c->slots, c->flags);
    return update_timing_begin(c, &I->timed);
}
static int pcg1_end(PcgRun &R, const Pcg1Iter &I, double bytes_per_row_less = 0.0) {
    PGD_TRY(update_timing_end(R.c, I.timed, ((I.lag == 1 ? 40.0 : 56.0) - bytes_per_row_less) * (double)R.n));
    PGD_LAUNCH_CHECK(R.c);
    return PGD_OK;
}

static int pcg_iter_two_launch(PcgRun &R, int k) {
    Pcg1Iter I;
    const int par = k & 1;
    PGD_TRY(pcg1_begin(R, k, R.p, true, false, &I));
    k_pcg1_step<<<R.g2v, TPB, 0, R.c->stream>>>(R.x, R.r, R.p, R.q, R.sc, R.n, I.prod, I.nparts, par ? R.part2 : R.part2b, R.g2v, par ? R.part2b : R.part2,
                                                 R.c->slots, R.c->flags, par, I.lag);
    return pcg1_end(R, I);
}

static int pcg_iter_single_sync(PcgRun &R, int k) {
    Pcg1Iter I;
    PGD_TRY(pcg1_begin(R, k, R.p, true, true, &I));
    launch_pcg1_update(R.c, R.g2v, R.x, R.r, R.p, R.q, R.sc, 0, R.n, S1_ALPHA, S1_BETA, R.part2, I.lag, 0, -1, nullptr);
    return pcg1_end(R, I);
}

static int pcg_iter_single_sync_recompute(PcgRun &R, int k) {
    Pcg1Iter I;
    double *p_cur = (k & 1) ? R.q : R.p, *p_next = (k & 1) ? R.p : R.q;
    PGD_TRY(pcg1_begin(R, k, p_cur, false, true, &I));
    PGD_TRY(launch_stencil_update(R.c, R.m, R.o, p_cur, p_next, R.x, R.r, R.sc, R.part2, I.lag));
    return pcg1_end(R, I, 8.0);
}

static int pcg_enqueue(PcgRun &R, int start, int count) {
    for (int k = start; k < start + count; ++k) {
        R.c->prof_iter = k;
        switch (R.form) {
        case PGD_PCG_FORM_PRECOND: PGD_TRY(pcg_iter_precond(R, k)); break;
        case PGD_PCG_FORM_TEXTBOOK: PGD_TRY(pcg_iter_textbook(R, k)); break;
        case PGD_PCG_FORM_TWO_LAUNCH: PGD_TRY(pcg_iter_two_launch(R, k)); break;
        case PGD_PCG_FORM_FOLDED: PGD_TRY(pcg_iter_folded(R, k)); break;
        case PGD_PCG_FORM_SINGLE_SYNC: PGD_TRY(pcg_iter_single_sync(R, k)); break;
        case PGD_PCG_FORM_SINGLE_SYNC_RECOMPUTE: PGD_TRY(pcg_iter_single_sync_recompute(R, k)); break;
        case PGD_PCG_FORM_DEFERRED_X: PGD_TRY(pcg_iter_deferred_x(R, k)); break;
        case PGD_PCG_FORM_PLAIN: PGD_TRY(pcg_iter_plain(R, k)); break;
        }
    }
    return PGD_OK;
}

static int pcg_drive(PcgRun &R, int CE, int maxit, int f[4], int &enq, double *dbg) {
    Ctx *c = R.c;
    hipGraphExec_t gexec = nullptr;
    if (dbg) { (void)hipStreamSynchronize(c->stream); dbg[0] = host_now(); }
    if (maxit >= CE) {
        PGD_TRY(ensure_partials(c, std::max<int64_t>(4 * (int64_t)MAX_VEC_BLOCKS, 2 * ((R.n + 63) / 64) + 64)));
        PGD_TRY(ensure_work(c, 5, 4096));
        const bool prof_saved = c->prof;
        c->prof = false;
        hipGraph_t graph = nullptr;
        if (hipStreamBeginCapture(c->stream, hipStreamCaptureModeThreadLocal) == hipSuccess) {
            const int rc = pcg_enqueue(R, 0, CE);
            const hipError_t e = hipStreamEndCapture(c->stream, &graph);
            if (rc != PGD_OK || e != hipSuccess || !graph ||
                hipGraphInstantiate(&gexec, graph, nullptr, nullptr, 0) != hipSuccess)
                gexec = nullptr;
            if (graph) (void)hipGraphDestroy(graph);
            (void)hipGetLastError();
        }
        c->prof = prof_saved;
    }
    if (dbg) { dbg[1] = host_now(); dbg[3] = gexec ? 1.0 : 0.0; }
    int rc_loop = PGD_OK;
    auto issue = [&](int chunk) -> int {
        const bool eager_for_timing = c->prof && ((enq / CE) % PROF_EAGER_EVERY == 0);
        if (gexec && chunk == CE && !eager_for_timing) {
            if (hipGraphLaunch(gexec, c->stream) != hipSuccess) return fail(c, PGD_ERR_HIP, "pcg_solve: hipGraphLaunch failed");
            return PGD_OK;
        }
        return pcg_enqueue(R, enq, chunk);
    };
    if (c->pcg_pipeline && pcg_flag_snapshots(c) == PGD_OK) {
        auto snap = [&](int slot) -> hipError_t {
            hipError_t e = hipMemcpyAsync(c->flags_host + 4 * slot, c->flags, 4 * sizeof(int), hipMemcpyDeviceToHost, c->stream);
            if (e == hipSuccess) e = hipEventRecord(c->flag_ev[slot], c->stream);
            return e;
        };
        int cur = 0;
        hipError_t e = snap(0);
        while (e == hipSuccess) {
            const int chunk = (maxit - enq < CE) ? maxit - enq : CE;
            if (chunk > 0) {
                if ((rc_loop = issue(chunk)) != PGD_OK) break;
                enq += chunk;
                if ((e = snap(cur ^ 1)) != hipSuccess) break;
            }
            if ((e = hipEventSynchronize(c->flag_ev[cur])) != hipSuccess) break;
            for (int i = 0; i < 4; ++i) f[i] = c->flags_host[4 * cur + i];
            if (f[0] || chunk <= 0) break;
            cur ^= 1;
        }
        if (e != hipSuccess && rc_loop == PGD_OK) rc_loop = fail(c, PGD_ERR_HIP, "pcg_solve: %s", hipGetErrorString(e));
    } else {
        while (true) {
            hipError_t e = hipMemcpyAsync(f, c->flags, 4 * sizeof(int), hipMemcpyDeviceToHost, c->stream);
            if (e == hipSuccess) e = hipStreamSynchronize(c->stream);
            if (e != hipSuccess) { rc_loop = fail(c, PGD_ERR_HIP, "pcg_solve: %s", hipGetErrorString(e)); break; }
            if (f[0] || enq >= maxit) break;
            const int chunk = (maxit - enq < CE) ? maxit - enq : CE;
            if ((rc_loop = issue(chunk)) != PGD_OK) break;
            enq += chunk;
        }
    }
    if (dbg) { (void)hipStreamSynchronize(c->stream); dbg[2] = host_now(); }
    if (gexec) (void)hipGraphExecDestroy(gexec);
    return rc_loop;
}

static int pcg_finish(PcgRun &R, const int f[4], int *iters, double *relres) {
    Ctx *c = R.c;
    if (R.scaled) {
        const int g = grid_for(R.n);
        R.x_scaled = false;
        const bool pending = R.form == PGD_PCG_FORM_DEFERRED_X && f[0] != 0 && f[1] > 0;
        const bool lag_pending = R.lag_x && f[1] > 0 && ((f[1] - 1) & 1) == 0;
        const int last_par = f[1] > 0 ? (f[1] - 1) & 1 : 0;
        const bool two = R.form == PGD_PCG_FORM_TWO_LAUNCH;
        const double *p_live = R.form == PGD_PCG_FORM_SINGLE_SYNC_RECOMPUTE && (f[1] & 1) ? R.q : R.p;
        k_scale_out<<<g, TPB, 0, c->stream>>>(R.x, R.r, R.sc, R.n, c->partials, (pending || lag_pending) ? p_live : nullptr, c->slots,
                                              R.S_PAIR + 2 * (f[1] & 1), S_PQ, lag_pending ? 1 : 0,
                                              two ? S1F_ALPHA + last_par : S1_ALPHA, two ? S1F_BETA + last_par : S1_BETA);
        PGD_LAUNCH_CHECK(c);
        PGD_TRY(reduce_partials(c, c->partials, g, 1, S_TMP, -1, 0, 0));
        if (!R.virt) R.invalidate_slots();
    }
    PGD_LAUNCH_CHECK(c);
    double s[PGD_NSLOTS];
    PGD_HIP(c, hipMemcpyAsync(s, c->slots, sizeof s, hipMemcpyDeviceToHost, c->stream));
    PGD_HIP(c, hipStreamSynchronize(c->stream));
    if (R.precond == PGD_PCG_PRECOND_VMG) vmg_note_setup(c);
    if (R.precond == PGD_PCG_PRECOND_CMG) cmg_note_setup(c);
    if (iters) *iters = f[1];
    const double rr = R.scaled ? s[S_TMP] : (f[1] > 0) ? s[R.S_PAIR + 2 * ((f[1] - 1) & 1) + 1] : s[R.S_INIT + 1];
    const double bb = s[R.S_INIT + 2];
    if (relres) *relres = (bb > 0.0) ? sqrt(rr / bb) : 0.0;
    if (f[2] != 0) return fail(c, f[2], "pcg_solve: breakdown (NaN residual) after %d iterations", f[1]);
    return PGD_OK;
}

}

using namespace pgd;

extern "C" {

int pgd_op_combine(pgd_handle h, pgd_handle mh, const pgd_handle *atoms, const double *coefs, int n,
                   const int32_t *bc_dofs, int64_t nbc, pgd_handle *op) {
    PGD_CTX(c, h);
    Mesh *m = get_mesh(c, mh);
    if (!m || !atoms || !coefs || !op || n < 1 || nbc < 0 || (nbc > 0 && !bc_dofs))
        return fail(c, PGD_ERR_INVALID, "op_combine: invalid arguments");
    std::vector<Csr *> atom_objs((size_t)n);
    for (int t = 0; t < n; ++t) {
        Csr *a = get_csr(c, atoms[t]);
        if (!a || a->mesh != mh) return fail(c, PGD_ERR_INVALID, "op_combine: atom %d is not on this mesh", t);
        if (*op && atoms[t] == *op) return fail(c, PGD_ERR_INVALID, "op_combine: output aliases an input");
        atom_objs[t] = a;
    }
    const bool bc_known = nbc > 0 && m->bc_dev && m->bc_host.size() == (size_t)nbc &&
                          std::memcmp(m->bc_host.data(), bc_dofs, (size_t)nbc * sizeof(int32_t)) == 0;
    if (!bc_known)
        for (int64_t i = 0; i < nbc; ++i)
            if (bc_dofs[i] < 0 || bc_dofs[i] >= m->nv) return fail(c, PGD_ERR_INVALID, "op_combine: bc dof out of range");
    Csr *o = nullptr;
    if (*op) {
        o = get_csr(c, *op);
        if (!o || o->mesh != mh) return fail(c, PGD_ERR_INVALID, "op_combine: *op is not an operator on this mesh");
    } else {
        std::unique_ptr<Csr> a(new Csr);
        a->kind = Obj::CSR;
        a->mesh = mh;
        o = a.get();
        *op = put_obj(c, a.release());
    }
    o->dinv_valid = false;
    o->uvals_valid = false;
    o->vals_pending = false;
    o->version += 1;
    o->rec_atoms.assign(atoms, atoms + n);
    o->rec_coefs.assign(coefs, coefs + n);
    o->rec_serials.resize((size_t)n);
    o->rec_versions.resize((size_t)n);
    for (int t = 0; t < n; ++t) { o->rec_serials[(size_t)t] = atom_objs[t]->serial; o->rec_versions[(size_t)t] = atom_objs[t]->version; }
    if (o->rec_bc && o->rec_bc_bytes < (size_t)nbc * sizeof(int)) { dev_release(c, o->rec_bc, o->rec_bc_bytes); o->rec_bc = nullptr; }
    o->rec_nbc = nbc;
    {
        uint64_t hsig = 0x9e3779b97f4a7c15ull ^ (uint64_t)nbc;
        auto mix = [&](uint64_t v) { hsig = (hsig ^ v) * 0xff51afd7ed558ccdull; hsig ^= hsig >> 32; };
        const int64_t step = nbc > 4096 ? nbc / 4096 : 1;
        for (int64_t i = 0; i < nbc; i += step) mix((uint64_t)(uint32_t)bc_dofs[i]);
        if (nbc > 0) mix((uint64_t)(uint32_t)bc_dofs[nbc - 1]);
        for (int t = 0; t < n; ++t) mix(atom_objs[t]->serial);
        o->bc_sig = hsig ? hsig : 1;
    }
    const uint8_t *mask = nullptr;
    if (nbc > 0) {
        if (!o->rec_bc) {
            void *p;
            o->rec_bc_bytes = (size_t)nbc * sizeof(int);
            PGD_TRY(dev_alloc(c, &p, o->rec_bc_bytes));
// ... 217 lines not shown
```

### pgdrome_amd/csrc/pgd_spmv.hip

```cpp
#include <chrono>
#include <cstring>

#include "pgd_internal.h"
#include "pgd_dia_march.h"

#include <algorithm>

namespace pgd {

constexpr int SPMV_CAP = 4096;
constexpr int SPMV_VROUNDS = 8;
constexpr int SPMV_CROUNDS = 4;
constexpr int MAXY = 8;

struct SpmvArgs {
    const int *row_ptr, *cols;
    const double *vals, *x, *w;
    double *y, *partials;
    const int *flags;
    int row_begin, row_end;
};

typedef double d2_t __attribute__((ext_vector_type(2)));
typedef int i4_t __attribute__((ext_vector_type(4)));
// ... 897 lines not shown
        acc0 = fma(a5, xm[-1], acc0);
        acc0 = fma(a4, xm[0], acc0);
        acc0 = fma(T.LD37.x, xc[-DM_HX - 1], acc0);
        acc0 = fma(T.D26.x, xc[-DM_HX], acc0);
        acc0 = fma(T.L15.x, xc[-1], acc0);
        acc0 = fma(T.A40.y, xa, acc0);
        acc0 = fma(T.A15.x, xc[1], acc0);
        acc0 = fma(T.A26.x, xb, acc0);
        acc0 = fma(T.A37.x, xc[DM_HX + 1], acc0);
        acc0 = fma(T.A40.x, xp[0], acc0);
        acc0 = fma(T.A15.y, xp[1], acc0);
        acc0 = fma(T.A26.y, xp[DM_HX], acc0);
        acc0 = fma(T.A37.y, xp[DM_HX + 1], acc0);
        double acc1 = b7 * xm[-1];
        acc1 = fma(b6, xm[0], acc1);
        acc1 = fma(b5, xm[DM_HX - 1], acc1);
        acc1 = fma(b4, xm[DM_HX], acc1);
        acc1 = fma(T.L37.x, xc[-1], acc1);
        acc1 = fma(T.A26.x, xa, acc1);
        acc1 = fma(T.LB15.x, xc[DM_HX - 1], acc1);
        acc1 = fma(T.B40.y, xb, acc1);
        acc1 = fma(T.B15.x, xc[DM_HX + 1], acc1);
        acc1 = fma(T.B26.x, xc[2 * DM_HX], acc1);
        acc1 = fma(T.B37.x, xc[2 * DM_HX + 1], acc1);
        acc1 = fma(T.B40.x, xp[DM_HX], acc1);
        acc1 = fma(T.B15.y, xp[DM_HX + 1], acc1);
        acc1 = fma(T.B26.y, xp[2 * DM_HX], acc1);
        acc1 = fma(T.B37.y, xp[2 * DM_HX + 1], acc1);
        const bool on = z < zb;
        double *yz = A.y + P * (on ? z : za);
        if (NTY) {
            if (STORE && live0 && on) __builtin_nontemporal_store(acc0, yz + base0);
            if (STORE && live1 && on) __builtin_nontemporal_store(acc1, yz + base1);
        } else {
            if (STORE && live0 && on) yz[base0] = acc0;
            if (STORE && live1 && on) yz[base1] = acc1;
        }
        if (DOT) {
            const double d0 = (live0 && on) ? acc0 : 0.0, d1 = (live1 && on) ? acc1 : 0.0;
            dot = fma(d0, xa, dot); dot2 = fma(d0, d0, dot2);
            dot = fma(d1, xb, dot); dot2 = fma(d1, d1, dot2);
        }
        if (look) { a4 = T.A40.x; b6 = T.A26.y; b4 = T.B40.x; a5 = T.L15.y; b7 = T.L37.y; b5 = T.LB15.y; a6 = T.D26.y; a7 = T.LD37.y; }
        put(z + 2, rv, rk);
        fetch(z + 2 + D, rv, rk);
        lds_barrier();
    };
#pragma clang loop unroll(disable)
    for (int z = za; z < zb; z += D) {
#pragma unroll
        for (int s = 0; s < D; ++s) step(z + s, rr[s], kk[s]);
    }
    if (DOT) {
        for (int pass = 0; pass < (A.qq ? 2 : 1); ++pass) {
            const double sum = wave_sum(pass ? dot2 : dot);
            __syncthreads();
            if (lane == 0) s_red[wv] = sum;
            __syncthreads();
            if (tid == 0) A.partials[A.qq ? 2 * b + pass : b] = (s_red[0] + s_red[1]) + (s_red[2] + s_red[3]);
        }
    }
}

struct StencilArgs {
    const uint8_t *cls;
    double c[8];
    int ident;
    const double *x;
    double *y, *partials;
    const int *flags;
    int nx, ny, nz;
    int zv0, zv1;
    int zm0, zm1;
    int zs0, zs1;
    int z0, z1, zchunk, tiles_x, tiles_y;
    int qq;
    int whatif;
    const double *b;
    double w;
    double *ur = nullptr, *ux = nullptr;
    const double *us = nullptr;
    double *slots = nullptr;
    int lag = 0;
};

#if defined(PGD_STENCIL_TIMING) || defined(PGD_STENCIL_WHATIF)
#define PGD_ST_WHATIF(bit) (A.whatif & (bit))
#else
#define PGD_ST_WHATIF(bit) 0
#endif

typedef int st_v2i __attribute__((ext_vector_type(2)));

template <bool DOT, bool STORE, int D, bool NTY, int OCC, int EPI = 0, int RWT = 4>
__global__ __launch_bounds__(256, OCC) void k_spmv_stencil_march(StencilArgs A) {
    static_assert(RWT == 4 || RWT == 2, "rows per thread");
    constexpr int NT = 256, RW = RWT, PY = 4 * RW, HY = PY + 2;
    constexpr int NQ = RW + 1;
    constexpr int SLOT = NQ * NT;
    constexpr int OOB = (int)0x40000000;
    constexpr int AUX_ST = (NTY && EPI != 3) ? 2 : 0;
    constexpr int AUX_RX = (NTY && EPI == 3) ? 2 : 0;
    static_assert(EPI != 3 || (DOT && STORE), "the PCG update leaves its partial sums and stores the new direction");
    __shared__ double s_x[4 * SLOT];
    __shared__ double s_red[4];
    if (A.flags && A.flags[0]) return;
    double u_alpha = 0.0, u_beta = 0.0, u_alpha_p = 0.0, u_ibeta_p = 0.0;
    bool u_exact = false, u_skip_x = false, u_two = false;
    if (EPI == 3) {
        u_alpha = A.slots[S1_ALPHA];
        u_beta = A.slots[S1_BETA];
        u_exact = A.flags[3] != 0;
        u_skip_x = A.lag == 1 && u_beta >= LAG_MIN_BETA;
        u_two = A.lag == 2 && A.slots[S1_PEND] != 0.0;
        u_alpha_p = u_two ? A.slots[S1_ALPHA_PREV] : 0.0;
        u_ibeta_p = u_two ? 1.0 / A.slots[S1_BETA_PREV] : 0.0;
        if (A.lag == 1 && blockIdx.x == 0 && threadIdx.x == 0) A.slots[S1_PEND] = u_skip_x ? 1.0 : 0.0;
    }
    const int tid = threadIdx.x, lane = tid & 63, wv = tid >> 6;
    const int b = xcd_remap(blockIdx.x, gridDim.x);
    const int per_chunk = A.tiles_x * A.tiles_y;
    const int chunk = b / per_chunk, tile = b - chunk * per_chunk;
    const int ty = tile / A.tiles_x, tx = tile - ty * A.tiles_x;
    const int x0 = tx * 64, y0 = ty * PY;
    const int64_t P = (int64_t)A.nx * A.ny;
    const unsigned P8 = (unsigned)(P * 8);
    const int centre = (RW * wv + 1) * DM_HX + lane + 1;
    const int za = A.z0 + chunk * A.zchunk, zb = min(A.z1, za + A.zchunk);
    if (za >= zb) {
        if (DOT && tid == 0) { if (A.qq) { A.partials[2 * b] = 0.0; A.partials[2 * b + 1] = 0.0; } else A.partials[b] = 0.0; }
        return;
    }
    int lv[NQ], sv[RW], cell4;
    double m[RW];
    unsigned fix = 0;
    {
        const uint8_t *cz = A.cls + P * min(max(A.zm0, 0), A.nz - 1);
#pragma unroll
        for (int q = 0; q < NQ; ++q) {
            int lx, ly;
            if (q < RW) { lx = lane + 1; ly = RW * wv + q + 1; }
            else if (tid < DM_HX) { lx = tid; ly = 0; }
            else if (tid < 2 * DM_HX) { lx = tid - DM_HX; ly = HY - 1; }
            else if (tid < 2 * DM_HX + PY) { lx = 0; ly = tid - 2 * DM_HX + 1; }
            else { lx = DM_HX - 1; ly = tid - 2 * DM_HX - PY + 1; }
            const bool ring = q < RW || tid < 2 * DM_HX + 2 * PY;
            const int gx = x0 - 1 + lx, gy = y0 - 1 + ly;
            const bool in = ring && gx >= 0 && gx < A.nx && gy >= 0 && gy < A.ny;
            const int off = in ? gx + A.nx * gy : 0;
            const bool masked = in && A.ident >= 0 && (int)cz[off] == A.ident;
            if (q < RW) {
                lv[q] = in ? 8 * off : OOB;
                sv[q] = lv[q];
                m[q] = (in && !masked) ? 1.0 : 0.0;
                if (in && masked) fix |= 1u << q;
            } else {
                lv[q] = (in && !masked) ? 8 * off : OOB;
                cell4 = ring ? ly * DM_HX + lx : DM_HX * HY + (tid - (2 * DM_HX + 2 * PY));
            }
        }
    }
    bool fixr[RW];
#pragma unroll
    for (int r = 0; r < RW; ++r) fixr[r] = ((fix >> r) & 1u) != 0;
    const double c0 = A.c[0], c1 = A.c[1], c2 = A.c[2], c3 = A.c[3], c4 = A.c[4], c5 = A.c[5], c6 = A.c[6], c7 = A.c[7];
    double dot = 0.0, dot2 = 0.0;
    auto rsrc_of = [&](const double *plane_ptr, bool live) {
        return __builtin_amdgcn_make_buffer_rsrc(const_cast<double *>(plane_ptr), 0, live ? (int)P8 : 0, 0x00020000);
    };
    auto fetch = [&](const double *xz, bool live, double (&v)[NQ]) {
        if (PGD_ST_WHATIF(2)) return;
        const auto r = rsrc_of(xz, live);
#pragma unroll
        for (int q = 0; q < NQ; ++q) {
            const st_v2i t = __builtin_amdgcn_raw_buffer_load_b64(r, lv[q], 0, 0);
            v[q] = __builtin_bit_cast(double, t);
        }
    };
    const int zd0 = min(A.zv0, A.zs0), zd1 = max(A.zv1, A.zs1);
    auto fetch_live = [&](int z) { return z >= zd0 && z < zd1 && z <= zb; };
    auto stage_main = [&](int zz, const double (&v)[NQ], double (&own)[RW]) {
        double *dst = s_x + (zz & 3) * SLOT;
#pragma unroll
        for (int q = 0; q < RW; ++q) { dst[centre + q * DM_HX] = v[q] * m[q]; own[q] = v[q]; }
        dst[cell4] = v[RW];
    };
    auto stage = [&](int zz, const double (&v)[NQ], double (&own)[RW]) {
        if (zz >= A.zs0 && zz < A.zs1) { stage_main(zz, v, own); return; }
        double *dst = s_x + (zz & 3) * SLOT;
#pragma unroll
        for (int q = 0; q < RW; ++q) { dst[centre + q * DM_HX] = 0.0; own[q] = v[q]; }
        dst[cell4] = 0.0;
    };
    const double *xq = A.x + P * (int64_t)(za - 1);
    double *yq = A.y + P * (int64_t)(za - 1);
    const double *bq = EPI == 2 ? A.b + P * (int64_t)za : nullptr;
    double rr[D][NQ];
    double own[3][RW];
    static_assert(D % 3 == 0, "the ring of own values rotates by name: the march is unrolled in multiples of three steps");
    {
        double t0[NQ], t1[NQ], t2[NQ];
        fetch(xq, fetch_live(za - 1), t0); fetch(xq + P, fetch_live(za), t1); fetch(xq + 2 * P, fetch_live(za + 1), t2);
        stage(za - 1, t0, own[2]); stage(za, t1, own[0]); stage(za + 1, t2, own[1]);
    }
    xq += 3 * P;
#pragma unroll
    for (int s = 0; s < D; ++s) { fetch(xq, fetch_live(za + 2 + s), rr[s]); xq += P; }
    yq += P;
    __syncthreads();
#ifdef PGD_STENCIL_TIMING
    long long st_prev = 0;
    const int st_slot = b == 0 ? 0 : b == 100 ? 1 : b == 300 ? 2 : b == (int)gridDim.x - 1 ? 3 : -1;
    int st_n = 0;
#define PGD_ST_STAMP(k)                                                                                   \
    do {                                                                                                  \
        if (st_slot >= 0 && tid == 0 && st_n < 48 * 4) {                                                  \
            long long t_;                                                                                 \
            asm volatile("s_memtime %0\n\ts_waitcnt lgkmcnt(0)" : "=s"(t_)::"memory");                   \
            A.partials[4096 + st_slot * 256 + st_n] = (double)(t_ - st_prev);                             \
            st_prev = t_;                                                                                 \
            st_n += 1;                                                                                    \
        }                                                                                                 \
    } while (0)
#else
#define PGD_ST_STAMP(k) do { } while (0)
#endif
    auto upd_plane = [&](const double *base, const double *yz) {
        return reinterpret_cast<const double *>(reinterpret_cast<const char *>(base) + (reinterpret_cast<const char *>(yz) - reinterpret_cast<const char *>(A.y)));
    };
    auto upd_load = [&](const double *yz, double (&ur)[RW], double (&ux)[RW], double (&us)[RW]) {
        const auto dr = rsrc_of(upd_plane(A.ur, yz), true);
#pragma unroll
        for (int r = 0; r < RW; ++r) ur[r] = __builtin_bit_cast(double, __builtin_amdgcn_raw_buffer_load_b64(dr, sv[r], 0, AUX_RX));
        const auto dx = rsrc_of(upd_plane(A.ux, yz), !u_skip_x);
#pragma unroll
        for (int r = 0; r < RW; ++r) ux[r] = __builtin_bit_cast(double, __builtin_amdgcn_raw_buffer_load_b64(dx, sv[r], 0, AUX_RX));
        const auto ds = rsrc_of(upd_plane(A.us, yz), u_exact);
#pragma unroll
        for (int r = 0; r < RW; ++r) us[r] = __builtin_bit_cast(double, __builtin_amdgcn_raw_buffer_load_b64(ds, sv[r], 0, 0));
    };
    auto upd_rows = [&](double *yz, const double (&qv)[RW], const double (&xo)[RW], const double (&ur)[RW], const double (&ux)[RW],
                        const double (&us)[RW]) {
        const auto dp = rsrc_of(yz, true), dr = rsrc_of(upd_plane(A.ur, yz), true), dx = rsrc_of(upd_plane(A.ux, yz), !u_skip_x);
#pragma unroll
        for (int r = 0; r < RW; ++r) {
            const double pi = xo[r], r0 = ur[r];
            if (!u_skip_x) {
                double xi = ux[r];
                if (u_two) xi = fma(u_alpha_p, (pi - r0) * u_ibeta_p, xi);
                xi = fma(u_alpha, pi, xi);
                __builtin_amdgcn_raw_buffer_store_b64(__builtin_bit_cast(st_v2i, xi), dx, sv[r], 0, AUX_RX);
            }
            const double ri = fma(-u_alpha, qv[r], r0);
            const double pn = fma(u_beta, pi, ri);
            __builtin_amdgcn_raw_buffer_store_b64(__builtin_bit_cast(st_v2i, ri), dr, sv[r], 0, AUX_RX);
            __builtin_amdgcn_raw_buffer_store_b64(__builtin_bit_cast(st_v2i, pn), dp, sv[r], 0, 0);
            const bool in = sv[r] != OOB;
            const double t = in ? ri : 0.0;
            dot = fma(t, t, dot);
            if (u_exact) { const double ts = t / (in ? us[r] : 1.0); dot2 = fma(ts, ts, dot2); }
        }
    };
    auto rows = [&](int z, double *yz, bool live, const double (&xo)[RW]) {
        double bv[RW];
        double ur[RW], ux[RW], us[RW];
        if (EPI == 2) {
            const auto rb = rsrc_of(bq, live);
#pragma unroll
            for (int r = 0; r < RW; ++r) bv[r] = __builtin_bit_cast(double, __builtin_amdgcn_raw_buffer_load_b64(rb, sv[r], 0, 0));
        }
        if (EPI == 3) upd_load(yz, ur, ux, us);
        const double *xm = s_x + ((z - 1) & 3) * SLOT + centre;
        const double *xc = s_x + (z & 3) * SLOT + centre;
        const double *xp = s_x + ((z + 1) & 3) * SLOT + centre;
        double M[RW + 1][2], C[RW + 2][3], Q[RW + 1][2];
        double acc[RW];
        if (PGD_ST_WHATIF(4)) {
#pragma unroll
            for (int r = 0; r < RW; ++r) { acc[r] = c7; C[r + 1][1] = c6; }
        } else {
#pragma unroll
            for (int j = 0; j <= RW; ++j) { M[j][0] = xm[(j - 1) * DM_HX - 1]; M[j][1] = xm[(j - 1) * DM_HX]; }
#pragma unroll
            for (int j = 0; j <= RW + 1; ++j) {
                if (j <= RW) C[j][0] = xc[(j - 1) * DM_HX - 1];
                C[j][1] = xc[(j - 1) * DM_HX];
                if (j >= 1) C[j][2] = xc[(j - 1) * DM_HX + 1];
            }
#pragma unroll
            for (int j = 0; j <= RW; ++j) { Q[j][0] = xp[j * DM_HX]; Q[j][1] = xp[j * DM_HX + 1]; }
            __builtin_amdgcn_sched_barrier(0);
#pragma unroll
            for (int r = 0; r < RW; ++r) acc[r] = c7 * M[r][0];
#define PGD_ST_ROWS(cc, V)                           \
    _Pragma("unroll") for (int r = 0; r < RW; ++r) acc[r] = fma(cc, V, acc[r])
            PGD_ST_ROWS(c6, M[r][1]);
            PGD_ST_ROWS(c5, M[r + 1][0]);
            PGD_ST_ROWS(c4, M[r + 1][1]);
            PGD_ST_ROWS(c3, C[r][0]);
            PGD_ST_ROWS(c2, C[r][1]);
            PGD_ST_ROWS(c1, C[r + 1][0]);
            PGD_ST_ROWS(c0, C[r + 1][1]);
            PGD_ST_ROWS(c1, C[r + 1][2]);
            PGD_ST_ROWS(c2, C[r + 2][1]);
            PGD_ST_ROWS(c3, C[r + 2][2]);
            PGD_ST_ROWS(c4, Q[r][0]);
            PGD_ST_ROWS(c5, Q[r][1]);
            PGD_ST_ROWS(c6, Q[r + 1][0]);
            PGD_ST_ROWS(c7, Q[r + 1][1]);
#undef PGD_ST_ROWS
        }
        if (EPI == 3) {
            double qv[RW];
#pragma unroll
            for (int r = 0; r < RW; ++r) qv[r] = fixr[r] ? xo[r] : acc[r];
            upd_rows(yz, qv, xo, ur, ux, us);
            return;
        }
        const auto ry = rsrc_of(yz, live && STORE && !PGD_ST_WHATIF(1));
#pragma unroll
        for (int r = 0; r < RW; ++r) {
            const double ev = EPI == 0 ? acc[r] : EPI == 1 ? fma(-A.w, acc[r], xo[r]) : fma(A.w, bv[r] - acc[r], xo[r]);
            const double yv = fixr[r] ? xo[r] : ev;
            if (STORE) __builtin_amdgcn_raw_buffer_store_b64(__builtin_bit_cast(st_v2i, yv), ry, sv[r], 0, AUX_ST);
            if (DOT && EPI == 2) dot = fma(yv, bv[r], dot);
            else if (DOT) {
                dot = fma(yv, xo[r], dot);
                const double t = sv[r] != OOB ? yv : 0.0;
                dot2 = fma(t, t, dot2);
            }
        }
    };
    auto copy_rows = [&](double *yz, const double (&xo)[RW]) {
        if (EPI == 3) {
            double ur[RW], ux[RW], us[RW];
            upd_load(yz, ur, ux, us);
            upd_rows(yz, xo, xo, ur, ux, us);
            return;
        }
        const auto ry = rsrc_of(yz, STORE);
#pragma unroll
        for (int r = 0; r < RW; ++r) {
            if (STORE) __builtin_amdgcn_raw_buffer_store_b64(__builtin_bit_cast(st_v2i, xo[r]), ry, sv[r], 0, AUX_ST);
            if (DOT && EPI == 0) { dot = fma(xo[r], xo[r], dot); dot2 = fma(xo[r], xo[r], dot2); }
        }
    };
    const bool pure = za - 1 >= A.zs0 && zb < A.zs1;
    int z = za;
    if (pure) {
#pragma clang loop unroll(disable)
        for (; z + D <= zb; z += D) {
#pragma unroll
            for (int s = 0; s < D; ++s) {
                rows(z + s, yq, true, own[s % 3]);
                PGD_ST_STAMP(0);
                stage_main(z + s + 2, rr[s], own[(s + 2) % 3]);
                PGD_ST_STAMP(1);
                fetch(xq, z + s + 2 + D <= zb, rr[s]);
                PGD_ST_STAMP(2);
                xq += P; yq += P;
                if (EPI == 2) bq += P;
                if (!PGD_ST_WHATIF(8)) lds_barrier();
                PGD_ST_STAMP(3);
            }
        }
    }
#pragma clang loop unroll(disable)
    for (; z < zb; z += D) {
#pragma unroll
        for (int s = 0; s < D; ++s) {
            const int zs = z + s;
            if (zs < zb) {
                if (zs >= A.zm0 && zs < A.zm1) rows(zs, yq, true, own[s % 3]);
                else if (zs >= A.zv0 && zs < A.zv1) copy_rows(yq, own[s % 3]);
            }
            stage(zs + 2, rr[s], own[(s + 2) % 3]);
            fetch(xq, fetch_live(zs + 2 + D), rr[s]);
            xq += P; yq += P;
            if (EPI == 2) bq += P;
            lds_barrier();
        }
    }
    if (EPI == 3 && !u_exact) dot2 = dot;
    if (DOT) {
        for (int pass = 0; pass < (A.qq ? 2 : 1); ++pass) {
            const double sum = wave_sum(pass ? dot2 : dot);
            __syncthreads();
            if (lane == 0) s_red[wv] = sum;
            __syncthreads();
            if (tid == 0) A.partials[A.qq ? 2 * b + pass : b] = (s_red[0] + s_red[1]) + (s_red[2] + s_red[3]);
        }
    }
}
#undef PGD_ST_STAMP
#undef PGD_ST_WHATIF

struct StencilInfo { int ok, ident, base, split; double c[8]; int zm0, zm1, g_lo, g_hi; };

__global__ void k_stencil_pick(const uint8_t *__restrict__ cls, double *__restrict__ table, const int *__restrict__ info,
                               int nx, int ny, int z_lo, int z_hi, StencilInfo *S) {
    if (threadIdx.x != 0 || blockIdx.x != 0) return;
    S->ok = 0; S->ident = -1; S->base = -1; S->split = 0;
    const int ncls = info[0];
    if (info[1] != 0 || ncls <= 0 || ncls >= CLS_MAX || z_hi <= z_lo) return;
    const int64_t mid = (int64_t)nx * ny * ((z_lo + z_hi) / 2) + (int64_t)nx * (ny / 2) + nx / 2;
    for (int k = 0; k < ncls; ++k) {
        bool id = table[k * 8 + cls_pos(0)] == 1.0;
        for (int s = 1; s < 8; ++s) id = id && table[k * 8 + cls_pos(s)] == 0.0;
        if (id) S->ident = k;
    }
    int base = cls[mid], best = -1;
    for (int k = 0; k < ncls; ++k) {
        int nzc = 0;
        for (int s = 1; s < 8; ++s) nzc += table[k * 8 + cls_pos(s)] != 0.0 ? 1 : 0;
        if (nzc > best || (nzc == best && k == (int)cls[mid])) { best = nzc; base = k; }
    }
    if (base == S->ident) return;
    S->base = base;
    for (int s = 0; s < 8; ++s) S->c[s] = table[base * 8 + cls_pos(s)];
    if (S->ident >= 0) {
// ... 922 lines not shown
                    else if (dot && store) k_spmv_stencil_march<true, true, 3, false, 2, 0, 2><<<wgs_s, 256, 0, c->stream>>>(F);
                    else if (dot) k_spmv_stencil_march<true, false, 3, false, 2, 0, 2><<<wgs_s, 256, 0, c->stream>>>(F);
                    else k_spmv_stencil_march<false, true, 3, false, 2, 0, 2><<<wgs_s, 256, 0, c->stream>>>(F);
                } else if (depth == 6) PGD_STENCIL(6, 2); else PGD_STENCIL(3, 2);
#undef PGD_STENCIL
                c->kcount[KC_STENCIL_MARCH] += 1;
                if (timed2) PGD_TRY(prof_end(c, m, nrows, store ? 16.0 : 8.0));
                PGD_LAUNCH_CHECK(c);
                return PGD_OK;
            }
            PGD_TRY(not_virtual());
            if (coded) {
                DiacArgs E;
                E.cls = a->cls; E.same = a->cls_same; E.table = a->cls_table; E.ncls = a->cls_count; E.x = x; E.y = y; E.partials = D.partials; E.flags = flags;
                E.nx = D.nx; E.ny = D.ny; E.nz = D.nz; E.z0 = D.z0; E.z1 = D.z1; E.zchunk = zchunk_c; E.tiles_x = D.tiles_x; E.tiles_y = D.tiles_y;
                E.qq = D.qq;
                E.nt_y = (D.qq && c->pcg_stream_hints) ? 1 : 0;
                if (nparts_out) *nparts_out = wgs_c;
                if (dot) PGD_TRY(ensure_partials(c, std::max<int64_t>(c->partials_off + (D.qq ? 2 : 1) * (int64_t)wgs_c, 4 * MAX_VEC_BLOCKS)));
                E.partials = c->partials + c->partials_off;
                const bool six = zchunk_c >= 12 && zchunk_c % 6 == 0 && c->spmv_fetch_depth != 3;
#define PGD_DIAC(DD)                                                                                       \
    do {                                                                                                   \
        if (dot && store && E.nt_y) k_spmv_diac_march2<true, true, DD, true><<<wgs_c, 256, 0, c->stream>>>(E);   \
        else if (dot && store) k_spmv_diac_march2<true, true, DD, false><<<wgs_c, 256, 0, c->stream>>>(E);       \
        else if (dot) k_spmv_diac_march2<true, false, DD, false><<<wgs_c, 256, 0, c->stream>>>(E);               \
        else k_spmv_diac_march2<false, true, DD, false><<<wgs_c, 256, 0, c->stream>>>(E);                        \
    } while (0)
                if (six) PGD_DIAC(6); else PGD_DIAC(3);
#undef PGD_DIAC
                c->kcount[KC_DIAC_MARCH] += 1;
                if (timed2) PGD_TRY(prof_end(c, m, nrows, 17.0));
                PGD_LAUNCH_CHECK(c);
                return PGD_OK;
            }
            if (c->spmv_variant == 0 && c->dia_march3 && (int64_t)64 * D.n < ((int64_t)1 << 31) && plane < ((int64_t)1 << 27)) {
                if (dot && store) k_spmv_dia_march3<true, true><<<wgs, 256, 0, c->stream>>>(D);
                else if (dot) k_spmv_dia_march3<true, false><<<wgs, 256, 0, c->stream>>>(D);
                else k_spmv_dia_march3<false, true><<<wgs, 256, 0, c->stream>>>(D);
            } else if (c->spmv_variant == 0) {
                if (dot && store) k_spmv_dia_march2<true, true><<<wgs, 256, 0, c->stream>>>(D);
                else if (dot) k_spmv_dia_march2<true, false><<<wgs, 256, 0, c->stream>>>(D);
                else k_spmv_dia_march2<false, true><<<wgs, 256, 0, c->stream>>>(D);
            } else if (wy == 8) PGD_MARCH(8); else PGD_MARCH(4);
#undef PGD_MARCH
            c->kcount[KC_DIA_MARCH] += 1;
        } else {
            PGD_TRY(not_virtual());
            PGD_TRY(prof_begin(c, dot, store, &timed2));
            if (dot && store) k_spmv_dia_rows<true, true><<<nblk, 64, 0, c->stream>>>(D);
            else if (dot) k_spmv_dia_rows<true, false><<<nblk, 64, 0, c->stream>>>(D);
            else k_spmv_dia_rows<false, true><<<nblk, 64, 0, c->stream>>>(D);
            c->kcount[KC_DIA_ROWS] += 1;
        }
        if (timed2) PGD_TRY(prof_end(c, m, nrows, 8.0 * (D.unit_diag ? 7 : 8) + 16));
        PGD_LAUNCH_CHECK(c);
        return PGD_OK;
    }
    PGD_TRY(not_virtual());
    const int grid = nblk;
    bool timed = false;
    PGD_TRY(prof_begin(c, dot, store, &timed));
#define PGD_SYM_LAUNCH(D, S)                                                          \
    do {                                                                              \
        if (m->sym_w == 4) k_spmv_sym<D, S, 4><<<grid, 64, 0, c->stream>>>(A);        \
        else k_spmv_sym<D, S, 8><<<grid, 64, 0, c->stream>>>(A);                      \
    } while (0)
    if (dot && store) PGD_SYM_LAUNCH(true, true);
    else if (dot) PGD_SYM_LAUNCH(true, false);
    else PGD_SYM_LAUNCH(false, true);
#undef PGD_SYM_LAUNCH
    c->kcount[KC_SYM_ROWS] += 1;
    if (timed) PGD_TRY(prof_end(c, m, nrows, 8.0 * m->sym_w + 18));
    PGD_LAUNCH_CHECK(c);
    return PGD_OK;
}

int stencil_update_blocks(const Ctx *c, const Mesh *m) {
    const int64_t plane = (int64_t)m->sym_nx * m->sym_ny;
    return stencil_shape(c, m->sym_nx, m->sym_ny, (int)(m->nv / plane), 3).wgs;
}

int launch_stencil_update(Ctx *c, const Mesh *m, const Csr *a, const double *p_in, double *p_out, double *x, double *r, const double *s,
                          double *pairs, int lag) {
    if (!stencil_whole_grid(c, m, a) || !c->flags || p_in == p_out)
        return fail(c, PGD_ERR_INVALID, "stencil update: the operator's products do not run in the stencil march over the whole grid");
    const int64_t plane = (int64_t)m->sym_nx * m->sym_ny;
    const int nz = (int)(m->nv / plane);
    const StencilShape sh = stencil_shape(c, m->sym_nx, m->sym_ny, nz, 3);
    StencilArgs F;
    F.cls = a->cls; F.ident = a->st_ident; F.x = p_in; F.y = p_out; F.flags = c->flags;
    F.zv0 = a->st_z0; F.zv1 = a->st_z1; F.zm0 = a->st_zm0; F.zm1 = a->st_zm1;
    F.zs0 = a->st_zm0 - (a->st_g_lo ? 1 : 0); F.zs1 = a->st_zm1 + (a->st_g_hi ? 1 : 0);
    for (int s2 = 0; s2 < 8; ++s2) F.c[s2] = a->st_c[s2];
    F.nx = m->sym_nx; F.ny = m->sym_ny; F.nz = nz; F.z0 = 0; F.z1 = nz;
    F.tiles_x = sh.tiles_x; F.tiles_y = sh.tiles_y; F.zchunk = sh.zchunk;
    F.qq = 1; F.whatif = 0; F.b = nullptr; F.w = 0.0;
    F.partials = pairs;
    F.ur = r; F.ux = x; F.us = s; F.slots = c->slots; F.lag = lag;
    const bool nt = c->pcg_stream_hints != 0;
    if (sh.rows_per_thread == 2) {
        if (nt) k_spmv_stencil_march<true, true, 3, true, 2, 3, 2><<<sh.wgs, 256, 0, c->stream>>>(F);
        else k_spmv_stencil_march<true, true, 3, false, 2, 3, 2><<<sh.wgs, 256, 0, c->stream>>>(F);
    } else if (nt) k_spmv_stencil_march<true, true, 3, true, 2, 3><<<sh.wgs, 256, 0, c->stream>>>(F);
    else k_spmv_stencil_march<true, true, 3, false, 2, 3><<<sh.wgs, 256, 0, c->stream>>>(F);
    c->pcg_recompute_launches += 1;
    PGD_LAUNCH_CHECK(c);
    return PGD_OK;
}

constexpr int GRAM_MAXV = 17;
struct MultiDotArgs {
    const double *w, *b;
    const double *v[GRAM_MAXV];
    int nv;
    int64_t lo, hi;
    double *partials;
};

__global__ __launch_bounds__(TPB) void k_multidot(MultiDotArgs A) {
    __shared__ double s_red[4];
    double acc[GRAM_MAXV + 1];
#pragma unroll
    for (int m = 0; m <= GRAM_MAXV; ++m) acc[m] = 0.0;
    for (int64_t i = A.lo + (int64_t)blockIdx.x * TPB + threadIdx.x; i < A.hi; i += (int64_t)gridDim.x * TPB) {
        const double wi = A.w[i];
        double last = 0.0;
#pragma unroll
        for (int m = 0; m < GRAM_MAXV; ++m)
            if (m < A.nv) { last = A.v[m][i]; acc[m] = fma(last, wi, acc[m]); }
        acc[GRAM_MAXV] = fma(last, A.b[i], acc[GRAM_MAXV]);
    }
#pragma unroll
    for (int m = 0; m <= GRAM_MAXV; ++m) {
        if (m < A.nv || m == GRAM_MAXV) {
            const double sum = block_sum(acc[m], s_red);
            if (threadIdx.x == 0) A.partials[(int64_t)blockIdx.x * (A.nv + 1) + (m == GRAM_MAXV ? A.nv : m)] = sum;
        }
    }
}

constexpr int PAIR_MAXV = 16;
struct MultiDot2Args {
    const double *w0, *w1;
    const double *v[PAIR_MAXV];
    int nv;
    int64_t lo, hi;
    double *partials;
};

__global__ __launch_bounds__(TPB) void k_multidot2(MultiDot2Args A) {
    __shared__ double s_red[4];
    double a0[PAIR_MAXV], a1[PAIR_MAXV];
#pragma unroll
    for (int m = 0; m < PAIR_MAXV; ++m) a0[m] = a1[m] = 0.0;
    for (int64_t i = A.lo + (int64_t)blockIdx.x * TPB + threadIdx.x; i < A.hi; i += (int64_t)gridDim.x * TPB) {
        const double x0 = A.w0[i], x1 = A.w1[i];
#pragma unroll
        for (int m = 0; m < PAIR_MAXV; ++m)
            if (m < A.nv) { const double y = A.v[m][i]; a0[m] = fma(y, x0, a0[m]); a1[m] = fma(y, x1, a1[m]); }
    }
#pragma unroll
    for (int m = 0; m < PAIR_MAXV; ++m) {
        if (m < A.nv) {
            const double s0 = block_sum(a0[m], s_red);
            const double s1 = block_sum(a1[m], s_red);
            if (threadIdx.x == 0) {
                A.partials[(int64_t)blockIdx.x * (2 * A.nv) + m] = s0;
                A.partials[(int64_t)blockIdx.x * (2 * A.nv) + A.nv + m] = s1;
            }
        }
    }
}

constexpr int GRAM9 = 9, GRAM9_NV = GRAM9 * (GRAM9 + 1) / 2 + GRAM9;
struct Gram9Args {
    const double *v[GRAM9], *w[GRAM9], *b;
    int k;
    int64_t lo, hi;
    double *partials;
};

// ... 67 lines not shown
        k_spmv_multi<<<nblk, TPB, 0, c->stream>>>(A);
        c->kcount[KC_MULTI] += 1;
        PGD_LAUNCH_CHECK(c);
        PGD_TRY(reduce_partials(c, c->partials, nblk, cnt, S_TMP, -1, 0, 0));
        PGD_HIP(c, hipMemcpyAsync(out_host + first, c->slots + S_TMP, cnt * sizeof(double), hipMemcpyDeviceToHost, c->stream));
        PGD_HIP(c, hipStreamSynchronize(c->stream));
    }
    return PGD_OK;
}

}

using namespace pgd;

extern "C" {

#if defined(PGD_STENCIL_TIMING) || defined(PGD_STENCIL_WHATIF)
int pgd_debug_read_partials(pgd_handle h, double *out, int first, int count) {
    PGD_CTX(c, h);
    PGD_HIP(c, hipMemcpyAsync(out, c->partials + first, (size_t)count * sizeof(double), hipMemcpyDeviceToHost, c->stream));
    PGD_HIP(c, hipStreamSynchronize(c->stream));
    return PGD_OK;
}
#endif

int pgd_classify_counts(pgd_handle h, int64_t *full, int64_t *cached) {
    PGD_CTX(c, h);
    if (full) *full = c->cls_full;
    if (cached) *cached = c->cls_fast;
    return PGD_OK;
}

int pgd_tune(pgd_handle h, int knob, int64_t value) {
    PGD_CTX(c, h);
    if (knob == PGD_TUNE_SPMV_ROWS && (value == 64 || value == 128 || value == 256)) { c->spmv_rows = (int)value; return PGD_OK; }
    if (knob == PGD_TUNE_SPMV_DICT && value >= 0 && value <= 2) { c->spmv_dict = (int)value; return PGD_OK; }
    if (knob == PGD_TUNE_SPMV_SYM && value >= 0 && value <= 1) { c->spmv_sym = (int)value; return PGD_OK; }
    if (knob == PGD_TUNE_SPMV_GRID_MIN_BYTES && value >= 0) { c->spmv_grid_min_plane_bytes = value; return PGD_OK; }
    if (knob == PGD_TUNE_SPMV_ZCHUNK_FORCE && value >= 0 && value <= 65536) { c->spmv_zchunk_force = (int)value; return PGD_OK; }
    if (knob == PGD_TUNE_PCG_FOLD_REDUCE && value >= 0 && value <= 1) { c->pcg_fold_reduce = (int)value; return PGD_OK; }
    if (knob == PGD_TUNE_PCG_SCALED && value >= 0 && value <= 1) { c->pcg_scaled = (int)value; return PGD_OK; }
    if (knob == PGD_TUNE_SPMV_ZCHUNK && value >= 0 && value <= 65536) { c->spmv_zchunk = (int)value; return PGD_OK; }
    if (knob == PGD_TUNE_PCG_SINGLE_SYNC && value >= 0 && value <= 1) { c->pcg_single_sync = (int)value; return PGD_OK; }
    if (knob == PGD_TUNE_UNIT_DIAG && value >= 0 && value <= 1) { c->spmv_unit_diag = (int)value; return PGD_OK; }
    if (knob == PGD_TUNE_PCG_DEFER_X && value >= 0 && value <= 1) { c->pcg_defer_x = (int)value; return PGD_OK; }
    if (knob == PGD_TUNE_FAULT_ITERATION && value >= -1 && value <= (1 << 30)) { c->fault_iteration = (int)value; return PGD_OK; }
    if (knob == PGD_TUNE_CLS_CACHE && value >= 0 && value <= 1) { c->cls_cache_on = (int)value; return PGD_OK; }
    if (knob == PGD_TUNE_SPMV_STENCIL && value >= 0 && value <= 1) { c->spmv_stencil = (int)value; return PGD_OK; }
    if (knob == PGD_TUNE_SPMV_ZCHUNK_STENCIL && value >= 0 && value <= 1024) { c->spmv_zchunk_stencil = (int)value; return PGD_OK; }
    if (knob == PGD_TUNE_STENCIL_DEPTH && (value == 0 || value == 3 || value == 6)) { c->stencil_depth = (int)value; return PGD_OK; }
    if (knob == PGD_TUNE_STENCIL_WG_PER_CU && value >= 1 && value <= 8) { c->stencil_wg_per_cu = (int)value; return PGD_OK; }
    if (knob == PGD_TUNE_FAULT_STAGE && value >= 0 && value <= 4) { c->fault_stage = (int)value; return PGD_OK; }
    if (knob == PGD_TUNE_FAULT_STALL_MS && value >= 0 && value <= 20000) { c->fault_stall_ms = (int)value; return PGD_OK; }
    if (knob == PGD_TUNE_COMBINE_DIA && value >= 0 && value <= 1) { c->spmv_combine_dia = (int)value; return PGD_OK; }
    if (knob == PGD_TUNE_SPMV_VARIANT && value >= 0 && value <= 2) { c->spmv_variant = (int)value; return PGD_OK; }
    if (knob == PGD_TUNE_SPMV_ROW_CLASSES && value >= 0 && value <= 1) { c->spmv_classes = (int)value; return PGD_OK; }
    if (knob == PGD_TUNE_ASM_LATTICE && value >= 0 && value <= 3) { c->asm_lattice = (int)value; return PGD_OK; }
    if (knob == PGD_TUNE_PCG_LAG_X && value >= 0 && value <= 1) { c->pcg_lag_x = (int)value; return PGD_OK; }
    if (knob == PGD_TUNE_PCG_STREAM_HINTS && value >= 0 && value <= 1) { c->pcg_stream_hints = (int)value; return PGD_OK; }
    if (knob == PGD_TUNE_PCG_SMALL_SINGLE_SYNC && value >= 0 && value <= 1) { c->pcg_small_ss = (int)value; return PGD_OK; }
    if (knob == PGD_TUNE_PCG_SMALL_ROWS && value >= 0) { c->pcg_small_ss_rows = value; return PGD_OK; }
    if (knob == PGD_TUNE_SPMV_FETCH_DEPTH && (value == 3 || value == 6)) { c->spmv_fetch_depth = (int)value; return PGD_OK; }
    if (knob == PGD_TUNE_SPMV_ZCHUNK_CODED2 && value >= 0 && value <= 1020) { c->spmv_zchunk_coded2 = (int)value / 6 * 6; return PGD_OK; }
    if (knob == PGD_TUNE_PCG_PIPELINE && value >= 0 && value <= 1) { c->pcg_pipeline = (int)value; return PGD_OK; }
    if (knob == PGD_TUNE_PCG_EXACT_PHASE && value >= 0 && value <= 1) { c->pcg_exact_phase = (int)value; return PGD_OK; }
    if (knob == PGD_TUNE_PCG_FOLD_FINISH && value >= 0 && value <= 1) { c->pcg_fold_finish = (int)value; return PGD_OK; }
    if (knob == PGD_TUNE_ATOM_FAST && value >= 0 && value <= 1) { c->atom_fast = (int)value; return PGD_OK; }
    if (knob == PGD_TUNE_LAZY_CSR && value >= 0 && value <= 1) { c->lazy_csr = (int)value; return PGD_OK; }
    if (knob == PGD_TUNE_SPMV_ZCHUNK_CODED && value >= 3 && value <= 1024) { c->spmv_zchunk_coded = (int)value; return PGD_OK; }
    if (knob == PGD_TUNE_PCG_PRECOND && value >= 0 && value <= 3) { c->pcg_precond = (int)value; return PGD_OK; }
    if (knob == PGD_TUNE_PCG_DERIVE_SCALED && value >= 0 && value <= 1) { c->pcg_derive_scaled = (int)value; return PGD_OK; }
    if (knob == PGD_TUNE_COMM_SELF_PERIODIC && value >= 0 && value <= 1) { c->comm.self_periodic = value != 0; return PGD_OK; }
    if (knob == PGD_TUNE_HALO_OVERLAP_MIN_ROWS && value >= 0) { c->comm.overlap_min_rows = value; return PGD_OK; }
    if (knob == PGD_TUNE_SHARD_ONE_MARCH && value >= 0 && value <= 1) { c->shard_one_march = (int)value; return PGD_OK; }
    if (knob == PGD_TUNE_DIA_MARCH3 && value >= 0 && value <= 1) { c->dia_march3 = (int)value; return PGD_OK; }
    if (knob == PGD_TUNE_STENCIL_ROWS && (value == 0 || value == 2 || value == 4)) { c->stencil_rows = (int)value; return PGD_OK; }
    if (knob == PGD_TUNE_PUSH_IN_UPDATE && (value == 0 || value == 1)) { c->push_in_update = (int)value; return PGD_OK; }
    if (knob == PGD_TUNE_MG_CHUNK && value >= 2 && value <= 16 && value % 2 == 0) { c->mg_chunk = (int)value; return PGD_OK; }
    if (knob == PGD_TUNE_MG_MARCH_MIN && value >= 0 && value <= 1 << 20) { c->mg_march_min = (int)value; return PGD_OK; }
    if (knob == PGD_TUNE_EVAL_VARIANT && value >= 0 && value <= 1) { c->eval_variant = (int)value; return PGD_OK; }
    if (knob == PGD_TUNE_EVAL_GRID_MAX && value >= 0 && value <= 1 << 20) { c->eval_grid_max = (int)value; return PGD_OK; }
    if (knob == PGD_TUNE_EVAL_SAMPLE_CHUNK && value >= 0 && value <= 1024) { c->eval_chunk = (int)value; return PGD_OK; }
    if (knob == PGD_TUNE_PCG_RECOMPUTE_Q && value >= 0 && value <= 1) { c->pcg_recompute_q = (int)value; return PGD_OK; }
    if (knob == PGD_TUNE_BLOCK_STORAGE && value >= 0 && value <= 2) { c->block_storage = (int)value; return PGD_OK; }
    return fail(c, PGD_ERR_INVALID, "tune: unknown knob %d or value out of range", knob);
}

int pgd_spmv(pgd_handle h, pgd_handle ah, pgd_handle xh, pgd_handle yh, int64_t r0, int64_t r1) {
    PGD_CTX(c, h);
    Csr *a = get_csr(c, ah);
    Mesh *m = a ? get_mesh(c, a->mesh) : nullptr;
    Vec *x = get_vec(c, xh), *y = get_vec(c, yh);
    if (!a || !m || !x || !y || x->n != m->nv || y->n != m->nv || x == y)
        return fail(c, PGD_ERR_INVALID, "spmv: invalid handles, size mismatch or x aliases y");
    if (atom_fast_form(c, m, a, r0, r1)) return launch_spmv_op(c, m, a, x->d, y->d, nullptr, r0, r1, false, true, nullptr, nullptr);
    if (c->spmv_sym && c->atom_fast && m->sym_nx > 0 && !a->immutable && a->uvals && a->uvals_valid && !a->uvals_scaled && !a->st_virtual) {
        const int64_t plane = (int64_t)m->sym_nx * m->sym_ny;
        const int64_t q0 = r0 < 0 ? 0 : r0, q1 = r1 < 0 ? m->nv : r1;
        if (q0 >= 0 && q1 <= m->nv && q0 <= q1 && q0 % plane == 0 && q1 % plane == 0)
            return launch_spmv_op(c, m, a, x->d, y->d, nullptr, q0, q1, false, true, nullptr, nullptr);
    }
    PGD_TRY(ensure_vals(c, m, a));
    return launch_spmv(c, m, a->vals, x->d, y->d, nullptr, r0, r1, false, true, nullptr, nullptr);
}

int pgd_bilinear(pgd_handle h, pgd_handle ah, pgd_handle xh, pgd_handle yh, int64_t r0, int64_t r1, double *out) {
    PGD_CTX(c, h);
    Csr *a = get_csr(c, ah);
    Mesh *m = a ? get_mesh(c, a->mesh) : nullptr;
    Vec *x = get_vec(c, xh), *y = get_vec(c, yh);
    if (!a || !m || !x || !y || !out || x->n != m->nv || y->n != m->nv)
        return fail(c, PGD_ERR_INVALID, "bilinear: invalid handles or size mismatch");
    int nparts = 0;
    PGD_TRY(ensure_vals(c, m, a));
    PGD_TRY(launch_spmv(c, m, a->vals, y->d, nullptr, x->d, r0, r1, true, false, nullptr, &nparts));
    if (nparts == 0) { *out = 0.0; return PGD_OK; }
    PGD_TRY(reduce_partials(c, c->partials, nparts, 1, S_TMP, -1, 0, 0));
    PGD_HIP(c, hipMemcpyAsync(out, c->slots + S_TMP, sizeof(double), hipMemcpyDeviceToHost, c->stream));
    PGD_HIP(c, hipStreamSynchronize(c->stream));
    return PGD_OK;
}

int pgd_bilinear_many(pgd_handle h, pgd_handle ah, pgd_handle xh, const pgd_handle *yhs, int ny, int64_t r0,
                      int64_t r1, double *out) {
    PGD_CTX(c, h);
    Csr *a = get_csr(c, ah);
    Mesh *m = a ? get_mesh(c, a->mesh) : nullptr;
    Vec *x = get_vec(c, xh);
    if (!a || !m || !x || !out || ny < 0 || (ny > 0 && !yhs) || x->n != m->nv)
        return fail(c, PGD_ERR_INVALID, "bilinear_many: invalid handles or size mismatch");
    std::vector<const double *> ys((size_t)ny);
    for (int k = 0; k < ny; ++k) {
        Vec *y = get_vec(c, yhs[k]);
        if (!y || y->n != m->nv) return fail(c, PGD_ERR_INVALID, "bilinear_many: invalid vector %d", k);
        ys[k] = y->d;
    }
    if (ny == 0) return PGD_OK;
    PGD_TRY(ensure_vals(c, m, a));
    return launch_spmv_multi(c, m, a->vals, x->d, ys.data(), ny, r0, r1, out);
}

int pgd_op_symmetrize(pgd_handle h, pgd_handle ah, int *used) {
    PGD_CTX(c, h);
    Csr *a = get_csr(c, ah);
    Mesh *m = a ? get_mesh(c, a->mesh) : nullptr;
    if (!a || !m) return fail(c, PGD_ERR_INVALID, "op_symmetrize: invalid handle");
    bool usable = false;
    PGD_TRY(ensure_sym(c, m, a, &usable));
    if (used) *used = usable ? 1 : 0;
    return PGD_OK;
}

int pgd_atom_product_form(pgd_handle h, pgd_handle ah, int *form) {
    PGD_CTX(c, h);
    Csr *a = get_csr(c, ah);
    Mesh *m = a ? get_mesh(c, a->mesh) : nullptr;
    if (!a || !m || !form) return fail(c, PGD_ERR_INVALID, "atom_product_form: invalid handle");
    *form = 0;
    if (atom_fast_form(c, m, a, 0, m->nv)) *form = a->cls_count > 0 ? 2 : 1;
    return PGD_OK;
}

int pgd_op_classify(pgd_handle h, pgd_handle ah, int *classes) {
    PGD_CTX(c, h);
    Csr *a = get_csr(c, ah);
    Mesh *m = a ? get_mesh(c, a->mesh) : nullptr;
// ... 196 lines not shown
```

Before: 17.05.

## Fold PCG scalar finish into stencil march and use scalar Jacobi scale

```diff
diff --git a/include/pgd_amd.h b/include/pgd_amd.h
--- a/include/pgd_amd.h
+++ b/include/pgd_amd.h
@@ -195,6 +195,8 @@
                    pgd_handle fields);
 
 enum {
+    PGD_TUNE_PCG_SCALAR_S = 56,
+    PGD_TUNE_PCG_FOLD_MARCH = 55,
     PGD_TUNE_BLOCK_STORAGE = 54,
     PGD_TUNE_PCG_RECOMPUTE_Q = 53,
     PGD_TUNE_EVAL_SAMPLE_CHUNK = 52,
diff --git a/pgdrome_amd/_lib.py b/pgdrome_amd/_lib.py
--- a/pgdrome_amd/_lib.py
+++ b/pgdrome_amd/_lib.py
@@ -144,6 +144,7 @@
 EVAL_STATS, EVAL_ENVELOPE, EVAL_EXCEED, EVAL_FIELDS = 1, 2, 4, 8
 TUNE_EVAL_VARIANT, TUNE_EVAL_GRID_MAX, TUNE_EVAL_SAMPLE_CHUNK = 50, 51, 52
 TUNE_BLOCK_STORAGE = 54
+TUNE_PCG_FOLD_MARCH, TUNE_PCG_SCALAR_S = 55, 56
 BLOCK_F32, BLOCK_F64, BLOCK_MAXK = 0, 1, 64
 
 
diff --git a/pgdrome_amd/csrc/pgd_internal.h b/pgdrome_amd/csrc/pgd_internal.h
--- a/pgdrome_amd/csrc/pgd_internal.h
+++ b/pgdrome_amd/csrc/pgd_internal.h
@@ -25,6 +25,7 @@
 enum { S_PQ = 2, S_TOL2 = 5, S_DMIN = 7 , S_TMP = 8  };
 enum { S1_RZ = 24, S1_RR = 25, S1_ALPHA = 26, S1_BETA = 27, S1_PQ = 28, S1_QQ = 29,
        S1_ALPHA_PREV = 40, S1_BETA_PREV = 41, S1_PEND = 42 };
+enum { S1F_ALPHA = 44 , S1F_BETA = 46 , S1F_EXACT = 48  };
 constexpr double LAG_MIN_BETA = 0.01;
 
 struct Ctx;
@@ -227,6 +228,8 @@
     int pcg_lag_x = 1;
     int pcg_recompute_q = 1;
     int64_t pcg_recompute_launches = 0;
+    int pcg_fold_march = 0;
+    int pcg_scalar_s = 1;
     int asm_lattice = 1;
     int spmv_fetch_depth = 6;
     int spmv_zchunk_coded2 = 96;
@@ -361,9 +364,14 @@
 int dia_classify(Ctx *c, const Mesh *m, Csr *a, int zrange_lo = -1, int zrange_hi = -1);
 bool stencil_row_range(const Ctx *c, const Mesh *m, const Csr *a, int64_t r0, int64_t r1);
 bool stencil_whole_grid(const Ctx *c, const Mesh *m, const Csr *a);
+struct StencilFold {
+    const double *prod; int nprod;
+    const double *vec_in; int nvec;
+    int par;
+};
 int stencil_update_blocks(const Ctx *c, const Mesh *m);
 int launch_stencil_update(Ctx *c, const Mesh *m, const Csr *a, const double *p_in, double *p_out, double *x, double *r, const double *s,
-                          double *pairs, int lag);
+                          double *pairs, int lag, double s_free = 0.0, const StencilFold *fold = nullptr);
 int launch_stencil_pass(Ctx *c, const uint8_t *cls, int ident, const double cst[8], int nx, int ny, int nz, int zm0, int zm1,
                         const double *x, const double *b, double *y, double w, int epi, bool dot, int *nparts, int z0 = 0, int z1 = -1);
 bool mg_prepare(Ctx *c, const Mesh *m, const Csr *a);
@@ -451,6 +459,20 @@
     return v;
 }
 
+struct Pcg1Scalars { double alpha, beta; int exact, done, status; double pq, qq, rz, rr; };
+__device__ __forceinline__ void pcg1_local_step(Pcg1Scalars &S, const double *__restrict__ slots, int exact_cur) {
+    S.alpha = S.beta = 0.0; S.exact = exact_cur; S.done = 0; S.status = 0;
+    const double tol2 = slots[S_TOL2];
+    if (!(S.rz == S.rz) || !(S.pq == S.pq)) { S.done = 1; S.status = PGD_ERR_SINGULAR; return; }
+    if (exact_cur) { if (S.rr <= tol2) { S.done = 1; return; } }
+    else if (S.rz * slots[S_DMIN] <= 1e4 * tol2) S.exact = 1;
+    if (!(S.rz > 0.0)) { S.done = 1; return; }
+    S.alpha = S.rz / S.pq;
+    double rnew = S.alpha * S.alpha * S.qq - S.rz;
+    if (!(rnew > 0.0)) rnew = 0.0;
+    S.beta = rnew / S.rz;
+}
+
 template <int NW>
 __device__ __forceinline__ double block_sum_n(double v, double *s_red ) {
     v = wave_sum(v);
diff --git a/pgdrome_amd/csrc/pgd_pcg.hip b/pgdrome_amd/csrc/pgd_pcg.hip
--- a/pgdrome_amd/csrc/pgd_pcg.hip
+++ b/pgdrome_amd/csrc/pgd_pcg.hip
@@ -427,6 +427,7 @@
     const double dinv = 1.0 / A.c[0], si = sqrt(dinv);
     out[0] = unit ? 1.0 : A.c[0] * si * si;
     for (int s = 1; s < 8; ++s) { double v = A.c[s]; v *= si * si; out[s] = v; }
+    out[8] = si;
 }
 
 __global__ void k_dmin_slot(const unsigned long long *__restrict__ dmax_bits, double *__restrict__ slots, int *__restrict__ flags) {
@@ -552,7 +553,6 @@
     }
 }
 
-enum { S1F_ALPHA = 44 , S1F_BETA = 46 , S1F_EXACT = 48  };
 
 __device__ __forceinline__ void pcg1_finish(double *slots, int *flags, double pq, double qq, double rz, double rr, int slot_alpha,
                                             int slot_beta, bool keep_prev = false) {
@@ -778,8 +778,6 @@
     }
 }
 
-struct Pcg1Scalars { double alpha, beta; int exact, done, status; double pq, qq, rz, rr; };
-
 __device__ __forceinline__ Pcg1Scalars pcg1_wg_scalars(const double *__restrict__ prod, int nprod, const double *__restrict__ vecp, int nvec,
                                                        const double *__restrict__ slots, int exact_cur, double *s_w ) {
     typedef double d2 __attribute__((ext_vector_type(2)));
@@ -801,16 +799,7 @@
     __syncthreads();
     Pcg1Scalars S;
     S.pq = out[0]; S.qq = out[1]; S.rz = out[2]; S.rr = out[3];
-    S.alpha = S.beta = 0.0; S.exact = exact_cur; S.done = 0; S.status = 0;
-    const double tol2 = slots[S_TOL2];
-    if (!(S.rz == S.rz) || !(S.pq == S.pq)) { S.done = 1; S.status = PGD_ERR_SINGULAR; return S; }
-    if (exact_cur) { if (S.rr <= tol2) { S.done = 1; return S; } }
-    else if (S.rz * slots[S_DMIN] <= 1e4 * tol2) S.exact = 1;
-    if (!(S.rz > 0.0)) { S.done = 1; return S; }
-    S.alpha = S.rz / S.pq;
-    double rnew = S.alpha * S.alpha * S.qq - S.rz;
-    if (!(rnew > 0.0)) rnew = 0.0;
-    S.beta = rnew / S.rz;
+    pcg1_local_step(S, slots, exact_cur);
     return S;
 }
 
@@ -1291,6 +1280,8 @@
     bool scaled = false, lag_x = false;
     bool x_scaled = false;
     bool virt = false;
+    double s_free = 0.0;
+    bool fold_march = false;
     double st_saved[8] = {0, 0, 0, 0, 0, 0, 0, 0};
     ~PcgRun() {
         if (virt) {
@@ -1347,12 +1338,13 @@
     for (int s2 = 0; s2 < 8; ++s2) in.c[s2] = o->st_c[s2];
     k_stencil_derive<<<1, 1, 0, c->stream>>>(in, c->spmv_unit_diag, c->work[5] + 16);
     PGD_LAUNCH_CHECK(c);
-    double out8[8];
-    PGD_HIP(c, hipMemcpyAsync(out8, c->work[5] + 16, sizeof out8, hipMemcpyDeviceToHost, c->stream));
+    double out9[9];
+    PGD_HIP(c, hipMemcpyAsync(out9, c->work[5] + 16, sizeof out9, hipMemcpyDeviceToHost, c->stream));
     PGD_HIP(c, hipStreamSynchronize(c->stream));
-    for (double v : out8) if (!std::isfinite(v)) return PGD_OK;
-    for (int s2 = 0; s2 < 8; ++s2) { R.st_saved[s2] = o->st_c[s2]; o->st_c[s2] = out8[s2]; }
+    for (double v : out9) if (!std::isfinite(v)) return PGD_OK;
+    for (int s2 = 0; s2 < 8; ++s2) { R.st_saved[s2] = o->st_c[s2]; o->st_c[s2] = out9[s2]; }
     o->st_virtual = R.virt = true;
+    R.s_free = out9[8];
     return PGD_OK;
 }
 
@@ -1400,11 +1392,13 @@
     R.lag_x = c->pcg_lag_x && pcg_single_sync(R.form);
     R.g2v = grid_for((n + 1) / 2, TPB, (n > ((int64_t)1 << 20) && n <= c->pcg_small_ss_rows && c->pcg_small_ss) ? 512 : MAX_VEC_BLOCKS);
     R.gvec = R.form == PGD_PCG_FORM_SINGLE_SYNC_RECOMPUTE ? stencil_update_blocks(c, R.m) : R.g2v;
-    if (2 * (int64_t)R.gvec > 4 * (int64_t)MAX_VEC_BLOCKS) PGD_TRY(ensure_work(c, 6, 2 * (int64_t)R.gvec));
+    R.fold_march = R.form == PGD_PCG_FORM_SINGLE_SYNC_RECOMPUTE && c->pcg_fold_march;
+    const int64_t half = 2 * std::max<int64_t>(MAX_VEC_BLOCKS, R.fold_march ? R.gvec : 0);
+    PGD_TRY(ensure_work(c, 6, std::max<int64_t>(2 * half, 2 * (int64_t)R.gvec)));
     R.part2 = c->work[6];
-    R.part2b = R.part2 + 2 * (int64_t)MAX_VEC_BLOCKS;
+    R.part2b = R.part2 + half;
     if (!pcg_single_sync(R.form)) return PGD_OK;
-    const bool two = R.form == PGD_PCG_FORM_TWO_LAUNCH;
+    const bool two = R.form == PGD_PCG_FORM_TWO_LAUNCH || R.fold_march;
     k_pcg1_seed<<<8, TPB, 0, c->stream>>>(two ? R.part2b : R.part2, R.gvec, c->slots, R.S_INIT, R.S_INIT + 1);
     if (two) PGD_HIP(c, hipMemsetAsync(c->slots + S1F_ALPHA, 0, 6 * sizeof(double), c->stream));
     PGD_LAUNCH_CHECK(c);
@@ -1512,9 +1506,14 @@
 
 static int pcg_iter_single_sync_recompute(PcgRun &R, int k) {
     Pcg1Iter I;
-    double *p_cur = (k & 1) ? R.q : R.p, *p_next = (k & 1) ? R.p : R.q;
-    PGD_TRY(pcg1_begin(R, k, p_cur, false, true, &I));
-    PGD_TRY(launch_stencil_update(R.c, R.m, R.o, p_cur, p_next, R.x, R.r, R.sc, R.part2, I.lag));
+    const int par = k & 1;
+    double *p_cur = par ? R.q : R.p, *p_next = par ? R.p : R.q;
+    const double s_free = (R.virt && R.c->pcg_scalar_s) ? R.s_free : 0.0;
+    PGD_TRY(pcg1_begin(R, k, p_cur, false, !R.fold_march, &I));
+    if (R.fold_march) {
+        const StencilFold F{I.prod, I.nparts, par ? R.part2 : R.part2b, R.gvec, par};
+        PGD_TRY(launch_stencil_update(R.c, R.m, R.o, p_cur, p_next, R.x, R.r, R.sc, par ? R.part2b : R.part2, I.lag, s_free, &F));
+    } else PGD_TRY(launch_stencil_update(R.c, R.m, R.o, p_cur, p_next, R.x, R.r, R.sc, R.part2, I.lag, s_free));
     return pcg1_end(R, I, 8.0);
 }
 
@@ -1611,7 +1610,7 @@
         const bool pending = R.form == PGD_PCG_FORM_DEFERRED_X && f[0] != 0 && f[1] > 0;
         const bool lag_pending = R.lag_x && f[1] > 0 && ((f[1] - 1) & 1) == 0;
         const int last_par = f[1] > 0 ? (f[1] - 1) & 1 : 0;
-        const bool two = R.form == PGD_PCG_FORM_TWO_LAUNCH;
+        const bool two = R.form == PGD_PCG_FORM_TWO_LAUNCH || R.fold_march;
         const double *p_live = R.form == PGD_PCG_FORM_SINGLE_SYNC_RECOMPUTE && (f[1] & 1) ? R.q : R.p;
         k_scale_out<<<g, TPB, 0, c->stream>>>(R.x, R.r, R.sc, R.n, c->partials, (pending || lag_pending) ? p_live : nullptr, c->slots,
                                               R.S_PAIR + 2 * (f[1] & 1), S_PQ, lag_pending ? 1 : 0,
diff --git a/pgdrome_amd/csrc/pgd_spmv.hip b/pgdrome_amd/csrc/pgd_spmv.hip
--- a/pgdrome_amd/csrc/pgd_spmv.hip
+++ b/pgdrome_amd/csrc/pgd_spmv.hip
@@ -1003,7 +1003,39 @@
     const double *us = nullptr;
     double *slots = nullptr;
     int lag = 0;
+    double s_free = 0.0;
+    const double *fold_prod = nullptr, *fold_vec = nullptr;
+    int fold_nprod = 0, fold_nvec = 0, fold_par = -1;
+    int *fold_flags = nullptr;
 };
+
+__device__ __forceinline__ void pcg1_sums_like_scalars(const double *__restrict__ prod, int nprod, const double *__restrict__ vecp, int nvec,
+                                                       double (&w)[4]) {
+    typedef double d2 __attribute__((ext_vector_type(2)));
+    double a[4][8];
+#pragma unroll
+    for (int v = 0; v < 4; ++v)
+#pragma unroll
+        for (int u = 0; u < 8; ++u) a[v][u] = 0.0;
+    const int nmax = nprod > nvec ? nprod : nvec;
+    int i = threadIdx.x;
+    for (; i + 7 * 256 < nmax; i += 8 * 256) {
+#pragma unroll
+        for (int u = 0; u < 8; ++u) {
+            const int k = i + u * 256;
+            if (k < nprod) { const d2 t = *reinterpret_cast<const d2 *>(prod + 2 * (int64_t)k); a[0][u] += t.x; a[1][u] += t.y; }
+            if (k < nvec) { const d2 t = *reinterpret_cast<const d2 *>(vecp + 2 * (int64_t)k); a[2][u] += t.x; a[3][u] += t.y; }
+        }
+    }
+#pragma unroll
+    for (int u = 0; u < 7; ++u) {
+        const int k = i + u * 256;
+        if (k < nprod) { const d2 t = *reinterpret_cast<const d2 *>(prod + 2 * (int64_t)k); a[0][u] += t.x; a[1][u] += t.y; }
+        if (k < nvec) { const d2 t = *reinterpret_cast<const d2 *>(vecp + 2 * (int64_t)k); a[2][u] += t.x; a[3][u] += t.y; }
+    }
+#pragma unroll
+    for (int v = 0; v < 4; ++v) w[v] = wave_sum(((a[v][0] + a[v][1]) + (a[v][2] + a[v][3])) + ((a[v][4] + a[v][5]) + (a[v][6] + a[v][7])));
+}
 
 #if defined(PGD_STENCIL_TIMING) || defined(PGD_STENCIL_WHATIF)
 #define PGD_ST_WHATIF(bit) (A.whatif & (bit))
@@ -1025,10 +1057,18 @@
     static_assert(EPI != 3 || (DOT && STORE), "the PCG update leaves its partial sums and stores the new direction");
     __shared__ double s_x[4 * SLOT];
     __shared__ double s_red[4];
-    if (A.flags && A.flags[0]) return;
+    __shared__ double s_w[16];
+    __shared__ int s_done;
+    const bool fold = EPI == 3 && A.fold_par >= 0;
+    if (fold) {
+        if (threadIdx.x == 0) s_done = A.flags[0];
+        __syncthreads();
+        if (s_done) return;
+    } else if (A.flags && A.flags[0]) return;
     double u_alpha = 0.0, u_beta = 0.0, u_alpha_p = 0.0, u_ibeta_p = 0.0;
     bool u_exact = false, u_skip_x = false, u_two = false;
-    if (EPI == 3) {
+    const bool u_s_known = EPI == 3 && A.s_free > 0.0;
+    if (EPI == 3 && !fold) {
         u_alpha = A.slots[S1_ALPHA];
         u_beta = A.slots[S1_BETA];
         u_exact = A.flags[3] != 0;
@@ -1122,11 +1162,47 @@
     {
         double t0[NQ], t1[NQ], t2[NQ];
         fetch(xq, fetch_live(za - 1), t0); fetch(xq + P, fetch_live(za), t1); fetch(xq + 2 * P, fetch_live(za + 1), t2);
+        xq += 3 * P;
+        if (fold) {
+#pragma unroll
+            for (int s = 0; s < D; ++s) { fetch(xq, fetch_live(za + 2 + s), rr[s]); xq += P; }
+            const int par = A.fold_par;
+            const int exact_cur = A.slots[S1F_EXACT + (par ^ 1)] != 0.0;
+            u_two = A.lag == 2 && A.slots[S1_PEND] != 0.0;
+            u_alpha_p = u_two ? A.slots[S1F_ALPHA + (par ^ 1)] : 0.0;
+            u_ibeta_p = u_two ? 1.0 / A.slots[S1F_BETA + (par ^ 1)] : 0.0;
+            double w[4];
+            pcg1_sums_like_scalars(A.fold_prod, A.fold_nprod, A.fold_vec, A.fold_nvec, w);
+            if (lane == 0) {
+#pragma unroll
+                for (int v = 0; v < 4; ++v) s_w[4 * v + wv] = w[v];
+            }
+            __syncthreads();
+            Pcg1Scalars S;
+            S.pq = (s_w[0] + s_w[1]) + (s_w[2] + s_w[3]);
+            S.qq = (s_w[4] + s_w[5]) + (s_w[6] + s_w[7]);
+            S.rz = (s_w[8] + s_w[9]) + (s_w[10] + s_w[11]);
+            S.rr = (s_w[12] + s_w[13]) + (s_w[14] + s_w[15]);
+            pcg1_local_step(S, A.slots, exact_cur);
+            if (blockIdx.x == 0 && tid == 0) {
+                A.slots[S1_PQ] = S.pq; A.slots[S1_QQ] = S.qq; A.slots[S1_RZ] = S.rz; A.slots[S1_RR] = S.rr;
+                A.slots[S1F_EXACT + par] = S.exact ? 1.0 : 0.0;
+                A.fold_flags[3] = S.exact;
+                if (S.done) { if (S.status) A.fold_flags[2] = S.status; A.fold_flags[0] = 1; }
+                else { A.slots[S1F_ALPHA + par] = S.alpha; A.slots[S1F_BETA + par] = S.beta; A.fold_flags[1] += 1; }
+            }
+            if (S.done) return;
+            u_alpha = S.alpha; u_beta = S.beta;
+            u_exact = S.exact != 0;
+            u_skip_x = A.lag == 1 && u_beta >= LAG_MIN_BETA;
+            if (A.lag == 1 && blockIdx.x == 0 && tid == 0) A.slots[S1_PEND] = u_skip_x ? 1.0 : 0.0;
+        }
         stage(za - 1, t0, own[2]); stage(za, t1, own[0]); stage(za + 1, t2, own[1]);
     }
-    xq += 3 * P;
-#pragma unroll
-    for (int s = 0; s < D; ++s) { fetch(xq, fetch_live(za + 2 + s), rr[s]); xq += P; }
+    if (!fold) {
+#pragma unroll
+        for (int s = 0; s < D; ++s) { fetch(xq, fetch_live(za + 2 + s), rr[s]); xq += P; }
+    }
     yq += P;
     __syncthreads();
 #ifdef PGD_STENCIL_TIMING
@@ -1156,12 +1232,13 @@
         const auto dx = rsrc_of(upd_plane(A.ux, yz), !u_skip_x);
 #pragma unroll
         for (int r = 0; r < RW; ++r) ux[r] = __builtin_bit_cast(double, __builtin_amdgcn_raw_buffer_load_b64(dx, sv[r], 0, AUX_RX));
+        if (u_s_known) return;
         const auto ds = rsrc_of(upd_plane(A.us, yz), u_exact);
 #pragma unroll
         for (int r = 0; r < RW; ++r) us[r] = __builtin_bit_cast(double, __builtin_amdgcn_raw_buffer_load_b64(ds, sv[r], 0, 0));
     };
     auto upd_rows = [&](double *yz, const double (&qv)[RW], const double (&xo)[RW], const double (&ur)[RW], const double (&ux)[RW],
-                        const double (&us)[RW]) {
+                        const double (&us)[RW], unsigned ones) {
         const auto dp = rsrc_of(yz, true), dr = rsrc_of(upd_plane(A.ur, yz), true), dx = rsrc_of(upd_plane(A.ux, yz), !u_skip_x);
 #pragma unroll
         for (int r = 0; r < RW; ++r) {
@@ -1179,7 +1256,11 @@
             const bool in = sv[r] != OOB;
             const double t = in ? ri : 0.0;
             dot = fma(t, t, dot);
-            if (u_exact) { const double ts = t / (in ? us[r] : 1.0); dot2 = fma(ts, ts, dot2); }
+            if (u_exact) {
+                const double sr = u_s_known ? (((ones >> r) & 1u) ? 1.0 : A.s_free) : us[r];
+                const double ts = t / (in ? sr : 1.0);
+                dot2 = fma(ts, ts, dot2);
+            }
         }
     };
     auto rows = [&](int z, double *yz, bool live, const double (&xo)[RW]) {
@@ -1235,7 +1316,7 @@
             double qv[RW];
 #pragma unroll
             for (int r = 0; r < RW; ++r) qv[r] = fixr[r] ? xo[r] : acc[r];
-            upd_rows(yz, qv, xo, ur, ux, us);
+            upd_rows(yz, qv, xo, ur, ux, us, fix);
             return;
         }
         const auto ry = rsrc_of(yz, live && STORE && !PGD_ST_WHATIF(1));
@@ -1256,7 +1337,7 @@
         if (EPI == 3) {
             double ur[RW], ux[RW], us[RW];
             upd_load(yz, ur, ux, us);
-            upd_rows(yz, xo, xo, ur, ux, us);
+            upd_rows(yz, xo, xo, ur, ux, us, ~0u);
             return;
         }
         const auto ry = rsrc_of(yz, STORE);
@@ -2345,8 +2426,8 @@
 }
 
 int launch_stencil_update(Ctx *c, const Mesh *m, const Csr *a, const double *p_in, double *p_out, double *x, double *r, const double *s,
-                          double *pairs, int lag) {
-    if (!stencil_whole_grid(c, m, a) || !c->flags || p_in == p_out)
+                          double *pairs, int lag, double s_free, const StencilFold *fold) {
+    if (!stencil_whole_grid(c, m, a) || !c->flags || p_in == p_out || (fold && (fold->vec_in == pairs || !fold->prod || !fold->vec_in)))
         return fail(c, PGD_ERR_INVALID, "stencil update: the operator's products do not run in the stencil march over the whole grid");
     const int64_t plane = (int64_t)m->sym_nx * m->sym_ny;
     const int nz = (int)(m->nv / plane);
@@ -2361,6 +2442,11 @@
     F.qq = 1; F.whatif = 0; F.b = nullptr; F.w = 0.0;
     F.partials = pairs;
     F.ur = r; F.ux = x; F.us = s; F.slots = c->slots; F.lag = lag;
+    F.s_free = s_free;
+    if (fold) {
+        F.fold_prod = fold->prod; F.fold_nprod = fold->nprod; F.fold_vec = fold->vec_in; F.fold_nvec = fold->nvec;
+        F.fold_par = fold->par & 1; F.fold_flags = c->flags;
+    }
     const bool nt = c->pcg_stream_hints != 0;
     if (sh.rows_per_thread == 2) {
         if (nt) k_spmv_stencil_march<true, true, 3, true, 2, 3, 2><<<sh.wgs, 256, 0, c->stream>>>(F);
@@ -2594,6 +2680,8 @@
     if (knob == PGD_TUNE_EVAL_GRID_MAX && value >= 0 && value <= 1 << 20) { c->eval_grid_max = (int)value; return PGD_OK; }
     if (knob == PGD_TUNE_EVAL_SAMPLE_CHUNK && value >= 0 && value <= 1024) { c->eval_chunk = (int)value; return PGD_OK; }
     if (knob == PGD_TUNE_PCG_RECOMPUTE_Q && value >= 0 && value <= 1) { c->pcg_recompute_q = (int)value; return PGD_OK; }
+    if (knob == PGD_TUNE_PCG_FOLD_MARCH && value >= 0 && value <= 1) { c->pcg_fold_march = (int)value; return PGD_OK; }
+    if (knob == PGD_TUNE_PCG_SCALAR_S && value >= 0 && value <= 1) { c->pcg_scalar_s = (int)value; return PGD_OK; }
     if (knob == PGD_TUNE_BLOCK_STORAGE && value >= 0 && value <= 2) { c->block_storage = (int)value; return PGD_OK; }
     return fail(c, PGD_ERR_INVALID, "tune: unknown knob %d or value out of range", knob);
 }
```

Measured after the change: 18.33, median of 6. 1.07x the previous value.
